# mit-han-lab/duo-attention

Hardware: NVIDIA H100
Metric: decode tok/s @512K ctx (+ prefill tok/s @128K in `prefill`), Llama-3-8B, DuoAttention 50% retrieval heads (higher is better)
Workload: dtype bf16

## Files before the change

duo_attention_b200/_C.py:

```python
from __future__ import annotations

import ctypes as C
import os

_HERE = os.path.dirname(os.path.abspath(__file__))
LIB_PATH = os.environ.get("DUO_B200_LIB") or os.path.join(_HERE, "csrc", "libduo_b200.so")

DUO_OK, DUO_EINVAL, DUO_EOVERFLOW, DUO_ECUDA, DUO_EWORKSPACE = 0, -1, -2, -3, -4
DT_BF16, DT_FP16 = 0, 1
KV_SAME, KV_INT4 = 0, 1
ROPE_NONE, ROPE_HF, ROPE_FP32 = 0, 1, 2
ROPE_SKIP_Q = 0x100
DECODE_MAX_Q = 16
DECODE_MAX_Q_INT4 = 8
RAGGED_MAX_BATCH = 64

SYMBOLS = [
    "duo_layer_create", "duo_layer_destroy", "duo_workspace_bytes", "duo_rope_append", "duo_attention",
    "duo_attention_mma", "duo_decode_fused", "duo_decode_ragged", "duo_ragged_workspace_bytes",
    "duo_decode_ragged_int4", "duo_ragged_int4_workspace_bytes", "duo_layer_create_pooled", "duo_decode_ragged_pooled",
    "duo_ragged_state_advance", "duo_state_advance", "duo_state_set", "duo_stream_commit", "duo_quant_int4", "duo_dequant_int4", "duo_dequant_int4_bf16", "duo_add_rmsnorm", "duo_silu_mul",
    "duo_attention_partial", "duo_merge_partials", "duo_attention_seq", "duo_decode_fused_seq",
    "duo_seqcomm_data_bytes", "duo_seqcomm_flag_bytes", "duo_seqcomm_create", "duo_seqcomm_destroy", "duo_seq_merge",
    "duo_comm_data_bytes", "duo_comm_flag_bytes", "duo_comm_create", "duo_comm_destroy", "duo_allreduce_add_rmsnorm",
    "duo_last_error_string", "duo_version",
]


class LayerDesc(C.Structure):
    _fields_ = [
        ("full_k", C.c_void_p), ("full_v", C.c_void_p), ("ring_k", C.c_void_p), ("ring_v", C.c_void_p),
        ("full_k_scale", C.c_void_p), ("full_k_zero", C.c_void_p), ("full_v_scale", C.c_void_p),
        ("full_v_zero", C.c_void_p), ("ring_k_scale", C.c_void_p), ("ring_k_zero", C.c_void_p),
        ("ring_v_scale", C.c_void_p), ("ring_v_zero", C.c_void_p),
        ("full_cap", C.c_int64),
        ("batch", C.c_int32), ("n_full", C.c_int32), ("n_stream", C.c_int32), ("group", C.c_int32),
        ("head_dim", C.c_int32), ("sink", C.c_int32), ("recent", C.c_int32), ("stage_cap", C.c_int32),
        ("dtype", C.c_int32), ("kv_format", C.c_int32),
    ]


class CacheState(C.Structure):
    _fields_ = [("full_len", C.c_int64), ("total", C.c_int64), ("lo", C.c_int64), ("device_state", C.c_void_p),
                ("seq_rank", C.c_int32), ("seq_world", C.c_int32), ("seq_block", C.c_int32), ("seq_reserved", C.c_int32)]


class SeqCommDesc(C.Structure):
    _fields_ = [("data", C.c_void_p * 8), ("flags", C.c_void_p * 8), ("local_state", C.c_void_p),
                ("rank", C.c_int32), ("world", C.c_int32), ("max_rows", C.c_int32)]


class CommDesc(C.Structure):
    _fields_ = [("data", C.c_void_p * 8), ("flags", C.c_void_p * 8), ("local_state", C.c_void_p),
                ("rank", C.c_int32), ("world", C.c_int32), ("hidden", C.c_int32), ("max_rows", C.c_int32),
                ("dtype", C.c_int32)]


_lib = None


def load():
    global _lib
    if _lib is not None:
        return _lib
    if not os.path.exists(LIB_PATH):
        raise RuntimeError(
            f"{LIB_PATH} not found: the CUDA extension is mandatory (no fallback). Build it with "
            "`python -c 'import __graft_entry__ as g; g.build()'` or `make -C duo_attention_b200/csrc`."
        )
    lib = C.CDLL(LIB_PATH)
    vp, i32, i64, f32, sz = C.c_void_p, C.c_int32, C.c_int64, C.c_float, C.c_size_t
    lib.duo_layer_create.argtypes = [C.POINTER(LayerDesc), C.POINTER(vp)]
    lib.duo_layer_create.restype = C.c_int
    lib.duo_layer_create_pooled.argtypes = [C.POINTER(LayerDesc), i64, C.POINTER(vp)]
    lib.duo_layer_create_pooled.restype = C.c_int
    lib.duo_layer_destroy.argtypes = [vp]
    lib.duo_layer_destroy.restype = None
    lib.duo_workspace_bytes.argtypes = [i32, i32, i32, i32]
    lib.duo_workspace_bytes.restype = sz
    lib.duo_rope_append.argtypes = [vp, C.POINTER(CacheState), vp, i64, vp, vp, i32, i32, vp]
    lib.duo_rope_append.restype = C.c_int
    for name in ("duo_attention", "duo_attention_mma"):
        fn = getattr(lib, name)
        fn.argtypes = [vp, C.POINTER(CacheState), vp, i64, vp, i32, f32, vp, sz, vp]
        fn.restype = C.c_int
    lib.duo_decode_fused.argtypes = [vp, C.POINTER(CacheState), vp, i64, vp, vp, i32, vp, i32, f32, vp, sz, vp]
    lib.duo_decode_fused.restype = C.c_int
    for name in ("duo_decode_ragged", "duo_decode_ragged_int4"):
        fn = getattr(lib, name)
        fn.argtypes = [vp, vp, i64, vp, i64, vp, vp, i32, vp, i32, f32, vp, sz, vp]
        fn.restype = C.c_int
    lib.duo_decode_ragged_pooled.argtypes = [vp, vp, vp, i64, vp, i64, vp, vp, i32, vp, i32, f32, vp, sz, vp]
    lib.duo_decode_ragged_pooled.restype = C.c_int
    for name in ("duo_ragged_workspace_bytes", "duo_ragged_int4_workspace_bytes"):
        fn = getattr(lib, name)
        fn.argtypes = [i32, i32]
        fn.restype = sz
    lib.duo_ragged_state_advance.argtypes = [vp, i32, i32, i32, i32, vp]
    lib.duo_ragged_state_advance.restype = C.c_int
    lib.duo_state_advance.argtypes = [vp, i32, i32, i32, vp]
    lib.duo_state_advance.restype = C.c_int
    lib.duo_state_set.argtypes = [vp, i64, i64, i64, vp]
    lib.duo_state_set.restype = C.c_int
    lib.duo_stream_commit.argtypes = [vp, C.POINTER(CacheState), i32, vp]
    lib.duo_stream_commit.restype = C.c_int
    lib.duo_quant_int4.argtypes = [vp, i64, i64, vp, vp, vp, vp]
    lib.duo_quant_int4.restype = C.c_int
    for name in ("duo_dequant_int4", "duo_dequant_int4_bf16"):
        fn = getattr(lib, name)
        fn.argtypes = [vp, vp, vp, i64, vp, vp]
        fn.restype = C.c_int
    lib.duo_add_rmsnorm.argtypes = [vp, vp, vp, vp, vp, i64, i32, f32, i32, vp]
    lib.duo_add_rmsnorm.restype = C.c_int
    lib.duo_silu_mul.argtypes = [vp, vp, i64, i32, i32, vp]
    lib.duo_silu_mul.restype = C.c_int
    lib.duo_attention_partial.argtypes = [vp, i64, vp, i64, vp, vp, i32, f32, vp, sz, vp]
    lib.duo_attention_partial.restype = C.c_int
    lib.duo_attention_seq.argtypes = [vp, C.POINTER(CacheState), vp, i64, vp, vp, vp, i32, f32, vp, sz, vp]
    lib.duo_attention_seq.restype = C.c_int
    lib.duo_decode_fused_seq.argtypes = [vp, C.POINTER(CacheState), vp, i64, vp, vp, i32, vp, vp, vp, f32, vp, sz, vp]
    lib.duo_decode_fused_seq.restype = C.c_int
    lib.duo_seqcomm_data_bytes.argtypes = [i32, i32]
    lib.duo_seqcomm_data_bytes.restype = sz
    lib.duo_seqcomm_flag_bytes.argtypes = [i32, i32]
    lib.duo_seqcomm_flag_bytes.restype = sz
    lib.duo_seqcomm_create.argtypes = [C.POINTER(SeqCommDesc), C.POINTER(vp)]
    lib.duo_seqcomm_create.restype = C.c_int
    lib.duo_seqcomm_destroy.argtypes = [vp]
    lib.duo_seqcomm_destroy.restype = None
    lib.duo_seq_merge.argtypes = [vp, vp, vp, vp, i32, i32, i32, i32, vp]
    lib.duo_seq_merge.restype = C.c_int
    lib.duo_merge_partials.argtypes = [vp, vp, i32, i64, i32, i32, vp, i32, vp]
    lib.duo_merge_partials.restype = C.c_int
    lib.duo_comm_data_bytes.argtypes = [i32, i32, i32, i32]
    lib.duo_comm_data_bytes.restype = sz
    lib.duo_comm_flag_bytes.argtypes = [i32, i32]
    lib.duo_comm_flag_bytes.restype = sz
    lib.duo_comm_create.argtypes = [C.POINTER(CommDesc), C.POINTER(vp)]
    lib.duo_comm_create.restype = C.c_int
    lib.duo_comm_destroy.argtypes = [vp]
    lib.duo_comm_destroy.restype = None
    lib.duo_allreduce_add_rmsnorm.argtypes = [vp, vp, vp, vp, vp, vp, i32, f32, vp]
    lib.duo_allreduce_add_rmsnorm.restype = C.c_int
    lib.duo_last_error_string.argtypes = []
    lib.duo_last_error_string.restype = C.c_char_p
    lib.duo_version.argtypes = []
    lib.duo_version.restype = C.c_int
    _lib = lib
    return lib


def last_error() -> str:
    return load().duo_last_error_string().decode("utf-8", "replace")


def check(rc: int):
    if rc == DUO_OK:
        return
    msg = last_error()
    if rc == DUO_EOVERFLOW or rc == DUO_EINVAL:
        raise ValueError(msg)
    raise RuntimeError(f"libduo_b200 error {rc}: {msg}")
```

duo_attention_b200/csrc/api.cu:

```cuda
#include <cstdarg>
#include <cstdio>
#include <cstdlib>
#include <cstring>
#include <new>

#include "duo_common.cuh"

namespace duo {

int sm_count_current_device() {
  static int sms[64] = {0};
  int dev = 0;
  if (cudaGetDevice(&dev) != cudaSuccess) return 132;
  int& v = sms[dev & 63];
  if (v == 0) {
    int n = 132;
    if (cudaDeviceGetAttribute(&n, cudaDevAttrMultiProcessorCount, dev) != cudaSuccess || n < 1) n = 132;
    v = n;
  }
  return v;
}

static thread_local char g_err[512] = "";

void set_error(const char* fmt, ...) {
  va_list ap;
  va_start(ap, fmt);
  vsnprintf(g_err, sizeof(g_err), fmt, ap);
  va_end(ap);
}
int cuda_fail(cudaError_t e, const char* what) {
  set_error("CUDA error %d (%s) in %s", (int)e, cudaGetErrorString(e), what);
  return DUO_ECUDA;
}

size_t mma_workspace_bytes(int batch, int n_kv, int group, int max_q_len);
int launch_attn_mma(const duo_layer* L, const duo_cache_state* st, const void* q, long long q_row_stride, void* out,
                    int q_len, float scale, void* workspace, size_t workspace_bytes, cudaStream_t stream);
int launch_attn_int4(const duo_layer* L, const duo_cache_state* st, const void* q, long long q_row_stride, void* out,
                     int q_len, float scale, void* workspace, size_t workspace_bytes, cudaStream_t stream);
bool tc_prefill_supported(const duo_layer* L, const duo_cache_state* st, int q_len);
int launch_attn_tc(const duo_layer* L, const duo_cache_state* st, const void* q, long long q_row_stride, void* out,
                   int q_len, float scale, cudaStream_t stream);
int launch_rope_append(const duo_layer* L, const duo_cache_state* st, void* qkv, long long row_stride, const void* cos,
                       const void* sin, int rope_mode, int q_len, cudaStream_t stream);
int launch_stream_commit(const duo_layer* L, const duo_cache_state* st, int q_len, cudaStream_t stream);
int launch_quant_int4(const void* in, long long in_row_stride, long long rows, void* packed, void* scale, void* zero,
                      cudaStream_t stream);
int launch_state_advance(long long* st, int n, int sink, int recent, cudaStream_t stream);
int launch_state_set(long long* st, long long full_len, long long total, long long lo, cudaStream_t stream);
int launch_dequant_int4(const void* packed, const void* scale, const void* zero, long long rows, void* out,
                        cudaStream_t stream);
int launch_dequant_int4_bf16(const void* packed, const void* scale, const void* zero, long long rows, void* out,
                             cudaStream_t stream);

int launch_attn_mma_partial(const duo_layer* L, long long n_keys, const void* q, long long q_row_stride, float* out_o,
                            float* out_lse, int q_len, float scale, void* workspace, size_t workspace_bytes,
                            cudaStream_t stream);
int launch_attn_mma_seq(const duo_layer* L, const duo_cache_state* st, const void* q, long long q_row_stride, void* out,
                        float* part_o, float* part_lse, int q_len, float scale, void* workspace, size_t workspace_bytes,
                        cudaStream_t stream);
int launch_decode_fused(const duo_layer* L, const duo_cache_state* st, const void* qkv, long long row_stride,
                        const void* cos, const void* sin, int rope_mode, void* out, int q_len, float scale,
                        void* workspace, size_t workspace_bytes, cudaStream_t stream);
int launch_decode_fused_int4(const duo_layer* L, const duo_cache_state* st, const void* qkv, long long row_stride,
                             const void* cos, const void* sin, int rope_mode, void* out, int q_len, float scale,
                             void* workspace, size_t workspace_bytes, cudaStream_t stream);
int launch_decode_ragged(const duo_layer* L, const long long* row_state, const long long* row_geom, const void* qkv,
                         long long row_stride, const void* cos, const void* sin, int rope_mode, void* out, int q_len,
                         float scale, void* workspace, size_t workspace_bytes, cudaStream_t stream);
size_t ragged_workspace_bytes(int batch, int n_kv);
int launch_decode_ragged_int4(const duo_layer* L, const long long* row_state, const long long* row_geom,
                              const void* qkv, long long row_stride, const void* cos, const void* sin, int rope_mode,
                              void* out, int q_len, float scale, void* workspace, size_t workspace_bytes,
                              cudaStream_t stream);
size_t ragged_int4_workspace_bytes(int batch, int n_kv);
int launch_ragged_state_advance(long long* st, int batch, int n, int sink, int recent, cudaStream_t stream);
int launch_decode_fused_seq(const duo_layer* L, const duo_cache_state* st, const void* qkv, long long row_stride,
                            const void* cos, const void* sin, int rope_mode, void* out, float* part_o, float* part_lse,
                            float scale, void* workspace, size_t workspace_bytes, cudaStream_t stream);
int launch_merge_partials(const float* o_parts, const float* lse_parts, int n_parts, long long tokens, int heads_total,
                          int heads_used, void* out, int dtype, cudaStream_t stream);
int launch_add_rmsnorm(const void* x, const void* residual, const void* weight, void* out_norm, void* out_res,
                       long long rows, int hidden, float eps, int dtype, cudaStream_t stream);
int launch_silu_mul(const void* gate_up, void* out, long long rows, int inter, int dtype, cudaStream_t stream);

typedef CUresult (*EncodeTiledFn)(CUtensorMap*, CUtensorMapDataType, cuuint32_t, void*, const cuuint64_t*,
                                  const cuuint64_t*, const cuuint32_t*, const cuuint32_t*, CUtensorMapInterleave,
                                  CUtensorMapSwizzle, CUtensorMapL2promotion, CUtensorMapFloatOOBfill);

EncodeTiledFn get_encode_fn() {
  static EncodeTiledFn fn = nullptr;
  if (fn) return fn;
  void* p = nullptr;
  cudaDriverEntryPointQueryResult qres;
  cudaError_t e = cudaGetDriverEntryPoint("cuTensorMapEncodeTiled", &p, cudaEnableDefault, &qres);
  if (e != cudaSuccess || qres != cudaDriverEntryPointSuccess || p == nullptr) {
    set_error("cudaGetDriverEntryPoint(cuTensorMapEncodeTiled) failed: %s", cudaGetErrorString(e));
    cudaGetLastError();
    return nullptr;
  }
  fn = reinterpret_cast<EncodeTiledFn>(p);
  return fn;
}

static int encode_kv_map(CUtensorMap* m, void* base, int dtype, long long slots, long long heads, int box_rows) {
  EncodeTiledFn fn = get_encode_fn();
  if (!fn) return DUO_ECUDA;
  cuuint64_t dims[3] = {(cuuint64_t)kHeadDim, (cuuint64_t)slots, (cuuint64_t)heads};
  cuuint64_t strides[2] = {(cuuint64_t)kHeadDim * 2, (cuuint64_t)slots * kHeadDim * 2};
  cuuint32_t box[3] = {64, (cuuint32_t)box_rows, 1};
  cuuint32_t estr[3] = {1, 1, 1};
  CUresult r = fn(m, dtype == DUO_DT_BF16 ? CU_TENSOR_MAP_DATA_TYPE_BFLOAT16 : CU_TENSOR_MAP_DATA_TYPE_FLOAT16, 3, base,
                  dims, strides, box, estr, CU_TENSOR_MAP_INTERLEAVE_NONE, CU_TENSOR_MAP_SWIZZLE_128B,
                  CU_TENSOR_MAP_L2_PROMOTION_L2_256B, CU_TENSOR_MAP_FLOAT_OOB_FILL_NONE);
  if (r != CUDA_SUCCESS) {
    set_error("cuTensorMapEncodeTiled failed with CUresult %d (base=%p slots=%lld heads=%lld)", (int)r, base, slots,
              heads);
    return DUO_ECUDA;
  }
  return DUO_OK;
}

int stage_offset(const duo_layer_desc& d) {
  const int W = d.sink + d.recent;
  return d.kv_format == DUO_KV_INT4 ? (W + 63) / 64 * 64 : W;
}

}

using namespace duo;

extern "C" {

const char* duo_last_error_string(void) { return g_err; }
int duo_version(void) { return 100; }

static int create_layer(const duo_layer_desc* desc, int64_t pool_tokens, duo_layer** out) {
  *out = nullptr;
  if (desc->head_dim != kHeadDim) {
    set_error("duo_layer_create: head_dim %d unsupported (only 128)", desc->head_dim);
    return DUO_EINVAL;
  }
  if (desc->batch < 1 || desc->n_full < 0 || desc->n_stream < 0 || desc->group < 1 || desc->sink < 0 ||
      desc->recent < 1 || desc->stage_cap < 1 || desc->full_cap < 0) {
    set_error("duo_layer_create: bad geometry");
    return DUO_EINVAL;
  }
  if (desc->dtype != DUO_DT_BF16 && desc->dtype != DUO_DT_FP16) {
    set_error("duo_layer_create: bad dtype %d", desc->dtype);
    return DUO_EINVAL;
  }
  if (desc->kv_format == DUO_KV_INT4) {
    const long long ring_slots = (long long)stage_offset(*desc) + desc->stage_cap;
    if ((pool_tokens == 0 && desc->full_cap % 8 != 0) || ring_slots % 8 != 0) {
      set_error("duo_layer_create: INT4 caches need full_cap and ring slots (%lld) to be multiples of 8", ring_slots);
      return DUO_EINVAL;
    }
  }
  duo_layer* L = new (std::nothrow) duo_layer();
  if (!L) {
    set_error("duo_layer_create: out of host memory");
    return DUO_EINVAL;
  }
  L->d = *desc;
  L->has_full_maps = false;
  L->has_ring_maps = false;
  L->pool_tokens = pool_tokens;
  memset(&L->maps, 0, sizeof(L->maps));
  if (desc->kv_format == DUO_KV_SAME) {
    const long long ring_slots = (long long)desc->sink + desc->recent + desc->stage_cap;
    int rc = DUO_OK;
    const long long slots = pool_tokens ? pool_tokens * desc->n_full : desc->full_cap;
    if (desc->n_full > 0 && slots > 0) {
      const long long heads = pool_tokens ? 1 : (long long)desc->batch * desc->n_full;
      rc = encode_kv_map(&L->maps.full_k64, desc->full_k, desc->dtype, slots, heads, 64);
      if (!rc) rc = encode_kv_map(&L->maps.full_v64, desc->full_v, desc->dtype, slots, heads, 64);
      if (!rc) rc = encode_kv_map(&L->maps.full_k128, desc->full_k, desc->dtype, slots, heads, 128);
      if (!rc) rc = encode_kv_map(&L->maps.full_v128, desc->full_v, desc->dtype, slots, heads, 128);
      L->has_full_maps = (rc == DUO_OK);
    }
    if (!rc && desc->n_stream > 0) {
      const long long heads = (long long)desc->batch * desc->n_stream;
      rc = encode_kv_map(&L->maps.ring_k64, desc->ring_k, desc->dtype, ring_slots, heads, 64);
      if (!rc) rc = encode_kv_map(&L->maps.ring_v64, desc->ring_v, desc->dtype, ring_slots, heads, 64);
      if (!rc) rc = encode_kv_map(&L->maps.ring_k128, desc->ring_k, desc->dtype, ring_slots, heads, 128);
      if (!rc) rc = encode_kv_map(&L->maps.ring_v128, desc->ring_v, desc->dtype, ring_slots, heads, 128);
      L->has_ring_maps = (rc == DUO_OK);
    }
    if (rc) {
      delete L;
      return rc;
    }
  }
  *out = L;
  return DUO_OK;
}

int duo_layer_create(const duo_layer_desc* desc, duo_layer** out) {
  if (!desc || !out) {
    set_error("duo_layer_create: null argument");
    return DUO_EINVAL;
  }
  return create_layer(desc, 0, out);
}

int duo_layer_create_pooled(const duo_layer_desc* desc, int64_t pool_tokens, duo_layer** out) {
  if (!desc || !out) {
    set_error("duo_layer_create_pooled: null argument");
    return DUO_EINVAL;
  }
  *out = nullptr;
  if (pool_tokens < 128 || pool_tokens % 128 != 0) {
    set_error("duo_layer_create_pooled: pool_tokens %lld is not a positive multiple of 128", (long long)pool_tokens);
    return DUO_EINVAL;
  }
  if (desc->n_full > 0 && pool_tokens * desc->n_full > INT32_MAX) {
    set_error("duo_layer_create_pooled: pool of %lld tokens x %d retrieval heads exceeds the 32-bit TMA row coordinate",
              (long long)pool_tokens, desc->n_full);
    return DUO_EINVAL;
  }
  return create_layer(desc, pool_tokens, out);
}

void duo_layer_destroy(duo_layer* layer) { delete layer; }

size_t duo_workspace_bytes(int32_t batch, int32_t n_kv_heads, int32_t group, int32_t max_q_len) {
  return mma_workspace_bytes(batch, n_kv_heads, group, max_q_len);
}

static int check_chunk(const duo_layer* L, const duo_cache_state* st, int q_len, const char* who) {
  if (!L || !st) {
    set_error("%s: null layer/state", who);
    return DUO_EINVAL;
  }
  if (L->pool_tokens) {
    set_error("%s: a pooled ragged layer is decoded with duo_decode_ragged_pooled only", who);
    return DUO_EINVAL;
  }
  if (q_len < 1) {
    set_error("%s: q_len %d < 1", who, q_len);
    return DUO_EINVAL;
  }
  if (st->full_len < 0 || st->total < 0 || st->lo < 0) {
    set_error("%s: negative cache state", who);
    return DUO_EINVAL;
  }
  long long need = st->full_len + q_len;
  if (st->seq_world != 0) {
    if (st->seq_world < 2 || st->seq_world > 8 || st->seq_rank < 0 || st->seq_rank >= st->seq_world || st->seq_block < 1) {
      set_error("%s: bad sequence-shard descriptor (rank %d, world %d, block %d)", who, st->seq_rank, st->seq_world,
                st->seq_block);
      return DUO_EINVAL;
    }
    const long long round = (long long)st->seq_block * st->seq_world, rem = need % round;
    long long extra = rem - (long long)st->seq_rank * st->seq_block;
    extra = extra < 0 ? 0 : (extra > st->seq_block ? st->seq_block : extra);
    need = need / round * st->seq_block + extra;
  }
  if (L->d.n_full > 0 && need > L->d.full_cap) {
    set_error("Trying to put %d KVs into a cache with max size %lld, current size: %lld.", q_len,
              (long long)L->d.full_cap, (long long)st->full_len);
    return DUO_EOVERFLOW;
  }
  if (q_len > L->d.stage_cap) {
    set_error("%s: chunk of %d tokens exceeds the staging capacity %d", who, q_len, L->d.stage_cap);
    return DUO_EOVERFLOW;
  }
  return DUO_OK;
}

int duo_rope_append(const duo_layer* layer, const duo_cache_state* st, void* qkv, int64_t qkv_row_stride,
                    const void* cos, const void* sin, int32_t rope_mode, int32_t q_len, void* stream) {
  int rc = check_chunk(layer, st, q_len, "duo_rope_append");
  if (rc) return rc;
  if (!qkv || ((rope_mode & 0xff) != DUO_ROPE_NONE && (!cos || !sin))) {
    set_error("duo_rope_append: null buffer");
    return DUO_EINVAL;
  }
  if ((rope_mode & 0xff) < DUO_ROPE_NONE || (rope_mode & 0xff) > DUO_ROPE_FP32 || (rope_mode & ~(0xff | DUO_ROPE_SKIP_Q))) {
    set_error("duo_rope_append: bad rope_mode %d", rope_mode);
    return DUO_EINVAL;
  }
  if (qkv_row_stride % 4 != 0) {
    set_error("duo_rope_append: row stride must be a multiple of 4 elements");
    return DUO_EINVAL;
  }
  return launch_rope_append(layer, st, qkv, qkv_row_stride, cos, sin, rope_mode, q_len, (cudaStream_t)stream);
}

int duo_attention(const duo_layer* layer, const duo_cache_state* st, const void* q, int64_t q_row_stride, void* out,
                  int32_t q_len, float scale, void* workspace, size_t workspace_bytes, void* stream) {
  int rc = check_chunk(layer, st, q_len, "duo_attention");
  if (rc) return rc;
  if (!q || !out) {
    set_error("duo_attention: null buffer");
    return DUO_EINVAL;
  }
  if (st->seq_world != 0) {
    set_error("duo_attention: sequence-sharded caches are attended with duo_attention_seq");
    return DUO_EINVAL;
  }
  if (layer->d.kv_format == DUO_KV_INT4)
    return launch_attn_int4(layer, st, q, q_row_stride, out, q_len, scale, workspace, workspace_bytes,
                            (cudaStream_t)stream);
  if (st->device_state && q_len > DUO_DECODE_MAX_Q) {
    set_error("duo_attention: device_state is only supported for chunks of <= %d tokens", DUO_DECODE_MAX_Q);
    return DUO_EINVAL;
  }
  if (tc_prefill_supported(layer, st, q_len))
    return launch_attn_tc(layer, st, q, q_row_stride, out, q_len, scale, (cudaStream_t)stream);
  return launch_attn_mma(layer, st, q, q_row_stride, out, q_len, scale, workspace, workspace_bytes,
                         (cudaStream_t)stream);
}

static int check_decode_args(const char* who, bool outputs_ok, const void* qkv, int64_t qkv_row_stride, const void* cos,
                             const void* sin, int32_t rope_mode) {
  if (!outputs_ok || !qkv || (rope_mode != DUO_ROPE_NONE && (!cos || !sin))) {
    set_error("%s: null buffer", who);
    return DUO_EINVAL;
  }
  if (rope_mode < DUO_ROPE_NONE || rope_mode > DUO_ROPE_FP32) {
    set_error("%s: bad rope_mode %d", who, rope_mode);
    return DUO_EINVAL;
  }
  if (qkv_row_stride % 8 != 0 || (reinterpret_cast<uintptr_t>(qkv) & 15)) {
    set_error("%s: qkv rows must be 16-byte aligned (row stride a multiple of 8 elements)", who);
    return DUO_EINVAL;
  }
  return DUO_OK;
}

int duo_decode_fused(const duo_layer* layer, const duo_cache_state* st, const void* qkv, int64_t qkv_row_stride,
                     const void* cos, const void* sin, int32_t rope_mode, void* out, int32_t q_len, float scale,
                     void* workspace, size_t workspace_bytes, void* stream) {
  int rc = check_chunk(layer, st, q_len, "duo_decode_fused");
  if (!rc) rc = check_decode_args("duo_decode_fused", out != nullptr, qkv, qkv_row_stride, cos, sin, rope_mode);
  if (rc) return rc;
  const int max_rows = layer->d.kv_format == DUO_KV_INT4 ? DUO_DECODE_MAX_Q_INT4 : DUO_DECODE_MAX_Q;
  if (layer->d.group * q_len > max_rows || st->seq_world != 0) {
    set_error("duo_decode_fused: unsharded caches and group * q_len <= %d only (got group %d, q_len %d)", max_rows,
              layer->d.group, q_len);
    return DUO_EINVAL;
  }
  if (layer->d.kv_format == DUO_KV_INT4)
    return launch_decode_fused_int4(layer, st, qkv, qkv_row_stride, cos, sin, rope_mode, out, q_len, scale, workspace,
                                    workspace_bytes, (cudaStream_t)stream);
  return launch_decode_fused(layer, st, qkv, qkv_row_stride, cos, sin, rope_mode, out, q_len, scale, workspace,
                             workspace_bytes, (cudaStream_t)stream);
}

size_t duo_ragged_workspace_bytes(int32_t batch, int32_t n_kv_heads) {
  if (batch < 1 || batch > DUO_RAGGED_MAX_BATCH || n_kv_heads < 1) return 0;
  return ragged_workspace_bytes(batch, n_kv_heads);
}

size_t duo_ragged_int4_workspace_bytes(int32_t batch, int32_t n_kv_heads) {
  if (batch < 1 || batch > DUO_RAGGED_MAX_BATCH || n_kv_heads < 1) return 0;
  return ragged_int4_workspace_bytes(batch, n_kv_heads);
}

static int check_ragged_rows(const char* who, const duo_layer* layer, int32_t q_len, int max_rows) {
  if (layer->d.batch > DUO_RAGGED_MAX_BATCH) {
    set_error("%s: batch %d exceeds %d rows", who, layer->d.batch, DUO_RAGGED_MAX_BATCH);
    return DUO_EINVAL;
  }
  if (q_len < 1 || layer->d.group * q_len > max_rows) {
    set_error("%s: group * q_len <= %d only (got group %d, q_len %d)", who, max_rows, layer->d.group, q_len);
    return DUO_EINVAL;
  }
  return DUO_OK;
}

static int check_ragged_args(const char* who, const duo_layer* layer, int64_t max_full_len, int32_t q_len,
                             int max_rows) {
  if (int rc = check_ragged_rows(who, layer, q_len, max_rows)) return rc;
  if (max_full_len < 0) {
    set_error("%s: negative max_full_len", who);
    return DUO_EINVAL;
  }
  if (layer->d.n_full > 0 && max_full_len + q_len > layer->d.full_cap) {
    set_error("Trying to put %d KVs into a cache with max size %lld, current size: %lld.", q_len,
              (long long)layer->d.full_cap, (long long)max_full_len);
    return DUO_EOVERFLOW;
  }
  return DUO_OK;
}

int duo_decode_ragged(const duo_layer* layer, const int64_t* row_state, int64_t max_full_len, const void* qkv,
                      int64_t qkv_row_stride, const void* cos, const void* sin, int32_t rope_mode, void* out,
                      int32_t q_len, float scale, void* workspace, size_t workspace_bytes, void* stream) {
  if (!layer || !row_state) {
    set_error("duo_decode_ragged: null argument");
    return DUO_EINVAL;
  }
  if (layer->pool_tokens) {
    set_error("duo_decode_ragged: a pooled ragged layer is decoded with duo_decode_ragged_pooled");
    return DUO_EINVAL;
  }
  if (int rc = check_decode_args("duo_decode_ragged", out != nullptr, qkv, qkv_row_stride, cos, sin, rope_mode)) return rc;
  if (layer->d.kv_format != DUO_KV_SAME) {
    set_error("duo_decode_ragged: 16-bit KV only (INT4 caches are decoded with duo_decode_ragged_int4)");
    return DUO_EINVAL;
  }
  if (int rc = check_ragged_args("duo_decode_ragged", layer, max_full_len, q_len, DUO_DECODE_MAX_Q)) return rc;
  return launch_decode_ragged(layer, reinterpret_cast<const long long*>(row_state), nullptr, qkv, qkv_row_stride, cos,
                              sin, rope_mode, out, q_len, scale, workspace, workspace_bytes, (cudaStream_t)stream);
}

int duo_decode_ragged_int4(const duo_layer* layer, const int64_t* row_state, int64_t max_full_len, const void* qkv,
                           int64_t qkv_row_stride, const void* cos, const void* sin, int32_t rope_mode, void* out,
                           int32_t q_len, float scale, void* workspace, size_t workspace_bytes, void* stream) {
  if (!layer || !row_state) {
    set_error("duo_decode_ragged_int4: null argument");
    return DUO_EINVAL;
  }
  if (layer->pool_tokens) {
    set_error("duo_decode_ragged_int4: a pooled ragged layer is decoded with duo_decode_ragged_pooled");
    return DUO_EINVAL;
  }
  if (int rc = check_decode_args("duo_decode_ragged_int4", out != nullptr, qkv, qkv_row_stride, cos, sin, rope_mode))
    return rc;
  if (layer->d.kv_format != DUO_KV_INT4) {
    set_error("duo_decode_ragged_int4: INT4 caches only (16-bit caches are decoded with duo_decode_ragged)");
    return DUO_EINVAL;
  }
  if (int rc = check_ragged_args("duo_decode_ragged_int4", layer, max_full_len, q_len, DUO_DECODE_MAX_Q_INT4)) return rc;
  return launch_decode_ragged_int4(layer, reinterpret_cast<const long long*>(row_state), nullptr, qkv, qkv_row_stride,
                                   cos, sin, rope_mode, out, q_len, scale, workspace, workspace_bytes,
                                   (cudaStream_t)stream);
}

int duo_decode_ragged_pooled(const duo_layer* layer, const int64_t* row_state, const int64_t* row_geom,
                             int64_t min_room, const void* qkv, int64_t qkv_row_stride, const void* cos,
                             const void* sin, int32_t rope_mode, void* out, int32_t q_len, float scale,
                             void* workspace, size_t workspace_bytes, void* stream) {
  const char* who = "duo_decode_ragged_pooled";
  if (!layer || !row_state || !row_geom) {
    set_error("%s: null argument", who);
    return DUO_EINVAL;
  }
  if (int rc = check_decode_args(who, out != nullptr, qkv, qkv_row_stride, cos, sin, rope_mode)) return rc;
  if (!layer->pool_tokens) {
    set_error("%s: the layer has no retrieval pool (create it with duo_layer_create_pooled)", who);
    return DUO_EINVAL;
  }
  const bool int4 = layer->d.kv_format == DUO_KV_INT4;
  if (int rc = check_ragged_rows(who, layer, q_len, int4 ? DUO_DECODE_MAX_Q_INT4 : DUO_DECODE_MAX_Q)) return rc;
  if (layer->d.n_full > 0 && q_len > min_room) {
    set_error("Trying to put %d KVs into a cache row with room for %lld more (%s).", q_len, (long long)min_room, who);
    return DUO_EOVERFLOW;
  }
  const long long* rs = reinterpret_cast<const long long*>(row_state);
  const long long* rg = reinterpret_cast<const long long*>(row_geom);
  if (int4)
    return launch_decode_ragged_int4(layer, rs, rg, qkv, qkv_row_stride, cos, sin, rope_mode, out, q_len, scale,
                                     workspace, workspace_bytes, (cudaStream_t)stream);
  return launch_decode_ragged(layer, rs, rg, qkv, qkv_row_stride, cos, sin, rope_mode, out, q_len, scale, workspace,
                              workspace_bytes, (cudaStream_t)stream);
}

int duo_ragged_state_advance(int64_t* row_state, int32_t batch, int32_t n, int32_t sink, int32_t recent, void* stream) {
  if (!row_state || batch < 1 || batch > DUO_RAGGED_MAX_BATCH || n < 0 || recent < 1 || sink < 0) {
    set_error("duo_ragged_state_advance: bad argument");
    return DUO_EINVAL;
  }
  return launch_ragged_state_advance(reinterpret_cast<long long*>(row_state), batch, n, sink, recent,
                                     (cudaStream_t)stream);
}

int duo_decode_fused_seq(const duo_layer* layer, const duo_cache_state* st, const void* qkv, int64_t qkv_row_stride,
                         const void* cos, const void* sin, int32_t rope_mode, void* out, float* out_o, float* out_lse,
                         float scale, void* workspace, size_t workspace_bytes, void* stream) {
  int rc = check_chunk(layer, st, 1, "duo_decode_fused_seq");
  if (!rc)
    rc = check_decode_args("duo_decode_fused_seq", out && out_o && out_lse, qkv, qkv_row_stride, cos, sin, rope_mode);
  if (rc) return rc;
  if (st->seq_world < 2) {
    set_error("duo_decode_fused_seq: the cache state carries no sequence-shard descriptor");
    return DUO_EINVAL;
  }
  if (layer->d.kv_format != DUO_KV_SAME || layer->d.group > 16) {
    set_error("duo_decode_fused_seq: 16-bit caches and group <= 16 only");
    return DUO_EINVAL;
  }
  return launch_decode_fused_seq(layer, st, qkv, qkv_row_stride, cos, sin, rope_mode, out, out_o, out_lse, scale, workspace,
                                 workspace_bytes, (cudaStream_t)stream);
}

int duo_attention_mma(const duo_layer* layer, const duo_cache_state* st, const void* q, int64_t q_row_stride,
                      void* out, int32_t q_len, float scale, void* workspace, size_t workspace_bytes, void* stream) {
  int rc = check_chunk(layer, st, q_len, "duo_attention_mma");
  if (rc) return rc;
  if (layer->d.kv_format != DUO_KV_SAME) {
    set_error("duo_attention_mma: 16-bit KV only");
    return DUO_EINVAL;
  }
  return launch_attn_mma(layer, st, q, q_row_stride, out, q_len, scale, workspace, workspace_bytes,
                         (cudaStream_t)stream);
}

int duo_state_advance(int64_t* device_state, int32_t n, int32_t sink, int32_t recent, void* stream) {
  if (!device_state || n < 0 || recent < 1 || sink < 0) {
    set_error("duo_state_advance: bad argument");
    return DUO_EINVAL;
  }
  return launch_state_advance(reinterpret_cast<long long*>(device_state), n, sink, recent, (cudaStream_t)stream);
}

int duo_state_set(int64_t* device_state, int64_t full_len, int64_t total, int64_t lo, void* stream) {
  if (!device_state || full_len < 0 || total < 0 || lo < 0) {
    set_error("duo_state_set: bad argument");
    return DUO_EINVAL;
  }
  return launch_state_set(reinterpret_cast<long long*>(device_state), full_len, total, lo, (cudaStream_t)stream);
}

int duo_stream_commit(const duo_layer* layer, const duo_cache_state* st, int32_t q_len, void* stream) {
  int rc = check_chunk(layer, st, q_len, "duo_stream_commit");
  if (rc) return rc;
  return launch_stream_commit(layer, st, q_len, (cudaStream_t)stream);
}

int duo_quant_int4(const void* in, int64_t in_row_stride, int64_t rows, void* packed, void* scale, void* zero,
                   void* stream) {
  if (rows < 0 || (rows > 0 && (!in || !packed || !scale || !zero)) || in_row_stride % 4 != 0) {
    set_error("duo_quant_int4: bad argument");
    return DUO_EINVAL;
  }
  return launch_quant_int4(in, in_row_stride, rows, packed, scale, zero, (cudaStream_t)stream);
}

int duo_attention_partial(const duo_layer* layer, int64_t n_keys, const void* q, int64_t q_row_stride, float* out_o,
                          float* out_lse, int32_t q_len, float scale, void* workspace, size_t workspace_bytes,
                          void* stream) {
  if (!layer || !q || !out_o || !out_lse || n_keys < 0 || q_len < 1) {
    set_error("duo_attention_partial: bad argument");
    return DUO_EINVAL;
  }
  if (layer->pool_tokens) {
    set_error("duo_attention_partial: a pooled ragged layer is decoded with duo_decode_ragged_pooled only");
    return DUO_EINVAL;
  }
  if (layer->d.kv_format != DUO_KV_SAME || layer->d.group * q_len > 16) {
    set_error("duo_attention_partial: 16-bit caches and group * q_len <= 16 only (got group %d, q_len %d)",
              layer->d.group, q_len);
    return DUO_EINVAL;
  }
  if (layer->d.n_full > 0 && n_keys > layer->d.full_cap) {
    set_error("duo_attention_partial: n_keys %lld exceeds the cache capacity %lld", (long long)n_keys,
              (long long)layer->d.full_cap);
    return DUO_EOVERFLOW;
  }
  return launch_attn_mma_partial(layer, n_keys, q, q_row_stride, out_o, out_lse, q_len, scale, workspace,
                                 workspace_bytes, (cudaStream_t)stream);
}

int duo_attention_seq(const duo_layer* layer, const duo_cache_state* st, const void* q, int64_t q_row_stride, void* out,
                      float* out_o, float* out_lse, int32_t q_len, float scale, void* workspace, size_t workspace_bytes,
                      void* stream) {
  int rc = check_chunk(layer, st, q_len, "duo_attention_seq");
  if (rc) return rc;
  if (!q || !out || !out_o || !out_lse) {
    set_error("duo_attention_seq: null buffer");
    return DUO_EINVAL;
  }
  if (st->seq_world < 2) {
    set_error("duo_attention_seq: the cache state carries no sequence-shard descriptor");
    return DUO_EINVAL;
  }
  if (layer->d.kv_format != DUO_KV_SAME || layer->d.group * q_len > 16) {
    set_error("duo_attention_seq: 16-bit caches and group * q_len <= 16 only (got group %d, q_len %d)", layer->d.group,
              q_len);
    return DUO_EINVAL;
  }
  return launch_attn_mma_seq(layer, st, q, q_row_stride, out, out_o, out_lse, q_len, scale, workspace, workspace_bytes,
                             (cudaStream_t)stream);
}

int duo_merge_partials(const float* o_parts, const float* lse_parts, int32_t n_parts, int64_t tokens,
                       int32_t heads_total, int32_t heads_used, void* out, int32_t dtype, void* stream) {
  if (n_parts < 1 || tokens < 0 || heads_total < 1 || heads_used < 0 || heads_used > heads_total ||
      (tokens > 0 && heads_used > 0 && (!o_parts || !lse_parts || !out)) ||
      (dtype != DUO_DT_BF16 && dtype != DUO_DT_FP16)) {
    set_error("duo_merge_partials: bad argument");
    return DUO_EINVAL;
  }
  return launch_merge_partials(o_parts, lse_parts, n_parts, tokens, heads_total, heads_used, out, dtype,
                               (cudaStream_t)stream);
}

int duo_add_rmsnorm(const void* x, const void* residual, const void* weight, void* out_norm, void* out_res, int64_t rows,
                    int32_t hidden, float eps, int32_t dtype, void* stream) {
  if (rows < 0 || hidden < 8 || hidden % 8 != 0 || hidden > 16384 || (rows > 0 && (!x || !weight || !out_norm)) ||
      (dtype != DUO_DT_BF16 && dtype != DUO_DT_FP16)) {
    set_error("duo_add_rmsnorm: bad argument");
    return DUO_EINVAL;
  }
  return launch_add_rmsnorm(x, residual, weight, out_norm, out_res, rows, hidden, eps, dtype, (cudaStream_t)stream);
}

int duo_silu_mul(const void* gate_up, void* out, int64_t rows, int32_t inter, int32_t dtype, void* stream) {
  if (rows < 0 || inter < 8 || inter % 8 != 0 || (rows > 0 && (!gate_up || !out)) ||
      (dtype != DUO_DT_BF16 && dtype != DUO_DT_FP16)) {
    set_error("duo_silu_mul: bad argument");
    return DUO_EINVAL;
  }
  return launch_silu_mul(gate_up, out, rows, inter, dtype, (cudaStream_t)stream);
}

int duo_dequant_int4(const void* packed, const void* scale, const void* zero, int64_t rows, void* out, void* stream) {
  if (rows < 0 || (rows > 0 && (!packed || !scale || !zero || !out))) {
    set_error("duo_dequant_int4: bad argument");
    return DUO_EINVAL;
  }
  return launch_dequant_int4(packed, scale, zero, rows, out, (cudaStream_t)stream);
}

int duo_dequant_int4_bf16(const void* packed, const void* scale, const void* zero, int64_t rows, void* out,
                          void* stream) {
  if (rows < 0 || (rows > 0 && (!packed || !scale || !zero || !out))) {
    set_error("duo_dequant_int4_bf16: bad argument");
    return DUO_EINVAL;
  }
  return launch_dequant_int4_bf16(packed, scale, zero, rows, out, (cudaStream_t)stream);
}

}
```

duo_attention_b200/csrc/attn_mma.cu:

```cuda
#include <type_traits>

#include "duo_common.cuh"

namespace duo {

constexpr int TILE = 64;
constexpr int STAGES = 3;
constexpr int KV_BOX_BYTES = TILE * 128;
constexpr int STAGE_BYTES = 4 * KV_BOX_BYTES;
constexpr int ATTN_THREADS = 128;

struct AttnParams {
  const void* q;
  void* out;
  long long q_tok_stride;
  long long q_batch_stride;
  long long out_batch_stride;
  int q_len, n_q_heads, group, n_full, n_stream, batch;
  int sink, recent, W;
  long long full_len, total, lo;
  const long long* dstate;
  float scale_log2;
  int splits_full;
  int keys_per_split;
  int n_rb;
  int cache_scan;
  SplitWs ws;
  float* part_o;
  float* part_lse;
  int no_causal;
  int seq_rank, seq_world, seq_block;
  const void* cos;
  const void* sin;
  int rope_mode;
  long long k_off, v_off;
  void *full_k, *full_v, *ring_k, *ring_v;
  long long full_cap;
  int ring_slots;
  int rg_slots;
  int rg_want;
  const long long* row_geom;
};


__host__ __device__ __forceinline__ long long seq_local_len(long long n, int rank, int world, int block) {
  const long long round = (long long)block * world;
  const long long full_rounds = n / round, rem = n % round;
  long long extra = rem - (long long)rank * block;
  extra = extra < 0 ? 0 : (extra > block ? block : extra);
  return full_rounds * block + extra;
}

template <typename T>
__device__ __forceinline__ void rope2(uint32_t& lo2, uint32_t& hi2, const void* cos, const void* sin, int mode, int tok,
                                      int d) {
  T* xl = reinterpret_cast<T*>(&lo2);
  T* xh = reinterpret_cast<T*>(&hi2);
#pragma unroll
  for (int e = 0; e < 2; ++e) {
    const float a = RopeCvt<T>::to_f(xl[e]), bb = RopeCvt<T>::to_f(xh[e]);
    float ol, oh;
    if (mode == DUO_ROPE_HF) {
      const T* ct = reinterpret_cast<const T*>(cos) + (long long)tok * kHeadDim;
      const T* st = reinterpret_cast<const T*>(sin) + (long long)tok * kHeadDim;
      ol = rope_hf<T>(a, -bb, RopeCvt<T>::to_f(ct[d + e]), RopeCvt<T>::to_f(st[d + e]));
      oh = rope_hf<T>(bb, a, RopeCvt<T>::to_f(ct[d + 64 + e]), RopeCvt<T>::to_f(st[d + 64 + e]));
    } else {
      const float* ct = reinterpret_cast<const float*>(cos) + (long long)tok * kHeadDim;
      const float* st = reinterpret_cast<const float*>(sin) + (long long)tok * kHeadDim;
      ol = rope_f32(a, -bb, ct[d + e], st[d + e]);
      oh = rope_f32(bb, a, ct[d + 64 + e], st[d + 64 + e]);
    }
    xl[e] = RopeCvt<T>::from_f(ol);
    xh[e] = RopeCvt<T>::from_f(oh);
  }
}

#ifdef DUO_TRACE
__device__ unsigned long long* g_duo_trace_mma = nullptr;
__device__ __forceinline__ void trace_stamp_mma(int slot) {
  if (threadIdx.x == 0 && g_duo_trace_mma) {
    unsigned long long t;
    asm volatile("mov.u64 %0, %%globaltimer;" : "=l"(t));
    g_duo_trace_mma[((long long)blockIdx.y * gridDim.x + blockIdx.x) * 4 + slot] = t;
  }
}
#define DUO_TRACE_MMA(slot) trace_stamp_mma(slot)
#else
#define DUO_TRACE_MMA(slot)
#endif

template <typename T, int KEY_WARPS, bool FUSED, bool RAGGED = false, bool POOLED = false>
__global__ void __launch_bounds__(ATTN_THREADS, 2)
duo_attn_mma_kernel(const __grid_constant__ CUtensorMap map_fk, const __grid_constant__ CUtensorMap map_fv,
                    const __grid_constant__ CUtensorMap map_rk, const __grid_constant__ CUtensorMap map_rv,
                    const AttnParams pin) {
  static_assert(!RAGGED || (FUSED && KEY_WARPS == 4), "the ragged variant is the fused decode kernel");
  static_assert(!POOLED || RAGGED, "the pooled layout is a ragged decode layout");
  DUO_TRACE_MMA(0);
  AttnParams p = pin;
  if (!RAGGED && pin.dstate) {
    p.full_len = pin.dstate[0];
    p.total = pin.dstate[1];
    p.lo = pin.dstate[2];
    const long long nk = p.seq_world > 1
                             ? seq_local_len(p.full_len + (FUSED ? 0 : p.q_len), p.seq_rank, p.seq_world, p.seq_block)
                             : p.full_len + (FUSED ? 0 : p.q_len);
    p.keys_per_split = (int)split_keys(nk, p.splits_full, TILE);
    p.cache_scan = (int)(p.total < p.W ? p.total : p.W);
  }
  constexpr int ROW_WARPS = 4 / KEY_WARPS;
  constexpr int ROWS = 16 * ROW_WARPS;
  constexpr int KPW = TILE / KEY_WARPS;
  constexpr int NT = KPW / 8;
  using Op = MmaOp<T>;

  extern __shared__ __align__(1024) uint8_t smem_raw[];
  uint8_t* smem = reinterpret_cast<uint8_t*>((reinterpret_cast<uintptr_t>(smem_raw) + 1023) & ~uintptr_t(1023));
  __shared__ uint64_t full_bar[STAGES];
  __shared__ int s_is_last;
  __shared__ float s_wmax[2][4][16];

  const int tid = threadIdx.x;
  const int warp = tid >> 5, lane = tid & 31;
  const int g = lane >> 2, t4 = lane & 3;
  int b = blockIdx.y;

  const int n_full_items = p.n_full * p.n_rb * p.splits_full;
  int kvh, rb, split;
  bool is_full;
  if constexpr (RAGGED) {
    const long long* rs = pin.dstate;
    rb = 0;
    split = 0;
    const int x = blockIdx.x, n_fslots = p.n_full * p.rg_slots;
    is_full = x < n_fslots;
    if (is_full) {
      const long long kps = ragged_batch_kps(rs, p.batch, 0, p.rg_want, TILE, 4 * TILE);
      kvh = x / p.rg_slots;
      const RaggedSlot s = ragged_slot(rs, p.batch, 0, kps, x % p.rg_slots);
      b = s.b;
      if (b == p.batch) return;
      split = s.split;
      p.keys_per_split = (int)kps;
      p.splits_full = s.splits;
      ragged_ws_slice<16>(p.ws, b, kvh, p.n_full, p.rg_slots, s);
    } else {
      const int y = x - n_fslots;
      b = y / p.n_stream;
      kvh = p.n_full + y % p.n_stream;
    }
    p.full_len = rs[4 * b];
    p.total = rs[4 * b + 1];
    p.lo = rs[4 * b + 2];
    p.cache_scan = (int)(p.total < p.W ? p.total : p.W);
    const long long tab = (long long)b * p.q_len * kHeadDim * (p.rope_mode == DUO_ROPE_HF ? (long long)sizeof(T) : 4);
    p.cos = reinterpret_cast<const uint8_t*>(p.cos) + tab;
    p.sin = reinterpret_cast<const uint8_t*>(p.sin) + tab;
  } else if ((int)blockIdx.x < n_full_items) {
    is_full = true;
    int x = blockIdx.x;
    split = x % p.splits_full;
    x /= p.splits_full;
    rb = p.n_rb - 1 - (x % p.n_rb);
    kvh = x / p.n_rb;
  } else {
    is_full = false;
    int x = blockIdx.x - n_full_items;
    rb = p.n_rb - 1 - (x % p.n_rb);
    kvh = p.n_full + x / p.n_rb;
    split = 0;
  }
  const int rows_total = p.group * p.q_len;
  const int row0 = rb * ROWS;
  const int rows_here = min(ROWS, rows_total - row0);
  const int tok_max = (row0 + rows_here - 1) / p.group;

  long long a0, a1, b0 = 0, b1 = 0;
  auto vis_count = [&](int t) -> long long {
    if (!is_full) return (long long)p.W + t + 1;
    if (p.no_causal) return p.full_len;
    if (p.seq_world > 1) return seq_local_len(p.full_len + t + 1, p.seq_rank, p.seq_world, p.seq_block);
    return p.full_len + t + 1;
  };
  bool has_new = false;
  long long new_base = 0;
  if (is_full) {
    const long long cached = p.seq_world > 1 ? seq_local_len(p.full_len, p.seq_rank, p.seq_world, p.seq_block) : p.full_len;
    const long long nkeys = FUSED ? cached : vis_count(tok_max);
    a0 = (long long)split * p.keys_per_split;
    a1 = min(nkeys, a0 + (long long)p.keys_per_split);
    if (a1 < a0) a1 = a0;
    has_new = FUSED && (split == p.splits_full - 1);
    if (FUSED && p.seq_world > 1)
      has_new = has_new && ((int)((p.full_len / p.seq_block) % p.seq_world) == p.seq_rank);
    new_base = cached;
  } else {
    a0 = 0;
    a1 = p.cache_scan;
    b0 = p.W;
    b1 = FUSED ? b0 : (long long)p.W + tok_max + 1;
    has_new = FUSED;
    new_base = p.W;
  }
  const int nA = (int)((a1 - a0 + TILE - 1) / TILE);
  const int nB = (int)((b1 - b0 + TILE - 1) / TILE);
  const int n_tiles = nA + nB;
  const int n_iter = n_tiles + (has_new ? 1 : 0);
  const CUtensorMap* mk = is_full ? &map_fk : &map_rk;
  const CUtensorMap* mv = is_full ? &map_fv : &map_rv;
  int pool_row0 = 0;
  if constexpr (POOLED) {
    if (is_full) pool_row0 = (int)(pin.row_geom[2 * b] * p.n_full + kvh * pin.row_geom[2 * b + 1]);
  }
  const int head_coord = (POOLED && is_full) ? 0 : is_full ? (b * p.n_full + kvh) : (b * p.n_stream + (kvh - p.n_full));

  if (tid == 0) {
    prefetch_tmap(mk);
    prefetch_tmap(mv);
    for (int s = 0; s < STAGES; ++s) mbar_init(&full_bar[s], 1);
    fence_barrier_init();
  }
  __syncthreads();

  auto tile_start = [&](int i) -> long long { return i < nA ? a0 + (long long)i * TILE : b0 + (long long)(i - nA) * TILE; };
  auto issue = [&](int i) {
    const int s = i % STAGES;
    uint8_t* dst = smem + s * STAGE_BYTES;
    const int j0 = (int)tile_start(i) + (POOLED ? pool_row0 : 0);
    mbar_expect_tx(&full_bar[s], STAGE_BYTES);
    tma_load_3d(dst, mk, &full_bar[s], 0, j0, head_coord);
    tma_load_3d(dst + KV_BOX_BYTES, mk, &full_bar[s], 64, j0, head_coord);
    tma_load_3d(dst + 2 * KV_BOX_BYTES, mv, &full_bar[s], 0, j0, head_coord);
    tma_load_3d(dst + 3 * KV_BOX_BYTES, mv, &full_bar[s], 64, j0, head_coord);
  };
  if (tid == 0) {
    for (int i = 0; i < STAGES - 1 && i < n_tiles; ++i) issue(i);
  }

  const int wrow = (KEY_WARPS == 1) ? warp * 16 : 0;
  const int wkey = (KEY_WARPS == 1) ? 0 : warp * KPW;
  uint32_t qa[8][4];
  int tok_r[2];
  {
    const T* qb = reinterpret_cast<const T*>(p.q) + (long long)b * p.q_batch_stride;
#pragma unroll
    for (int hf = 0; hf < 2; ++hf) {
      const int R = row0 + wrow + g + hf * 8;
      const bool ok = R < rows_total;
      const int tok = ok ? R / p.group : 0;
      const int hq = kvh * p.group + (ok ? R % p.group : 0);
      tok_r[hf] = ok ? tok : -1;
      const T* src = qb + (long long)tok * p.q_tok_stride + (long long)hq * kHeadDim;
#pragma unroll
      for (int kk = 0; kk < 8; ++kk) {
        uint32_t v0 = 0, v1 = 0;
        if (ok) {
          v0 = *reinterpret_cast<const uint32_t*>(src + kk * 16 + 2 * t4);
          v1 = *reinterpret_cast<const uint32_t*>(src + kk * 16 + 8 + 2 * t4);
        }
        qa[kk][hf] = v0;
        qa[kk][hf + 2] = v1;
      }
      if constexpr (FUSED) {
        if (ok && p.rope_mode != DUO_ROPE_NONE) {
#pragma unroll
          for (int kk = 0; kk < 4; ++kk) {
#pragma unroll
            for (int half = 0; half < 2; ++half) {
              const int d = kk * 16 + half * 8 + 2 * t4;
              rope2<T>(qa[kk][hf + 2 * half], qa[kk + 4][hf + 2 * half], p.cos, p.sin, p.rope_mode, tok, d);
            }
          }
        }
      }
    }
  }

  const long long lim_r[2] = {tok_r[0] >= 0 ? vis_count(tok_r[0]) : 0, tok_r[1] >= 0 ? vis_count(tok_r[1]) : 0};
  const long long lim_min = vis_count((row0 + wrow) / p.group);

  float o[16][4];
#pragma unroll
  for (int i = 0; i < 16; ++i) o[i][0] = o[i][1] = o[i][2] = o[i][3] = 0.f;
  float m_run[2] = {-INFINITY, -INFINITY};
  float l_run[2] = {0.f, 0.f};

  const int lrow = lane & 7;
  const int lmat = lane >> 3;

  for (int i = 0; i < n_iter; ++i) {
    __syncthreads();
    uint32_t sK;
    long long j0, jend;
    if (!FUSED || i < n_tiles) {
      if (tid == 0 && i + STAGES - 1 < n_tiles) issue(i + STAGES - 1);
      const int s = i % STAGES;
      mbar_wait(&full_bar[s], (i / STAGES) & 1);
      sK = smem_u32(smem + s * STAGE_BYTES);
      j0 = tile_start(i);
      jend = (i < nA) ? a1 : b1;
    } else {
      uint8_t* st0 = smem;
      for (int x = tid; x < STAGE_BYTES / 16; x += ATTN_THREADS) reinterpret_cast<uint4*>(st0)[x] = make_uint4(0, 0, 0, 0);
      __syncthreads();
      const T* rows = reinterpret_cast<const T*>(p.q) + (long long)b * p.q_batch_stride;
      auto dst_row = [&](int r) -> long long {
        if (is_full)
          return (POOLED ? (long long)pool_row0 : ((long long)b * p.n_full + kvh) * p.full_cap) + new_base + r;
        const long long pos = p.total + r;
        long long slot;
        if (pos < p.sink) slot = pos;
        else if (r >= p.q_len - p.recent) slot = p.sink + (pos - p.sink) % p.recent;
        else return -1;
        return ((long long)b * p.n_stream + (kvh - p.n_full)) * p.ring_slots + slot;
      };
      T* gk = reinterpret_cast<T*>(is_full ? p.full_k : p.ring_k);
      T* gv = reinterpret_cast<T*>(is_full ? p.full_v : p.ring_v);
      for (int w = tid; w < p.q_len * 8; w += ATTN_THREADS) {
        const int r = w >> 3, c = w & 7;
        const T* src = rows + (long long)r * p.q_tok_stride + p.k_off + (long long)kvh * kHeadDim;
        uint4 lo = *reinterpret_cast<const uint4*>(src + c * 8);
        uint4 hi = *reinterpret_cast<const uint4*>(src + 64 + c * 8);
        if (p.rope_mode != DUO_ROPE_NONE) rope8<T>(lo, hi, p.cos, p.sin, p.rope_mode, r, c * 8);
        const uint32_t off = r * 128 + ((c ^ (r & 7)) << 4);
        *reinterpret_cast<uint4*>(st0 + off) = lo;
        *reinterpret_cast<uint4*>(st0 + KV_BOX_BYTES + off) = hi;
        const long long dr = dst_row(r);
        if (dr >= 0) {
          *reinterpret_cast<uint4*>(gk + dr * kHeadDim + c * 8) = lo;
          *reinterpret_cast<uint4*>(gk + dr * kHeadDim + 64 + c * 8) = hi;
        }
      }
      for (int w = tid; w < p.q_len * 16; w += ATTN_THREADS) {
        const int r = w >> 4, c = w & 15;
        const T* src = rows + (long long)r * p.q_tok_stride + p.v_off + (long long)kvh * kHeadDim;
        const uint4 v = *reinterpret_cast<const uint4*>(src + c * 8);
        *reinterpret_cast<uint4*>(st0 + (2 + (c >> 3)) * KV_BOX_BYTES + r * 128 + (((c & 7) ^ (r & 7)) << 4)) = v;
        const long long dr = dst_row(r);
        if (dr >= 0) *reinterpret_cast<uint4*>(gv + dr * kHeadDim + c * 8) = v;
      }
      __syncthreads();
      sK = smem_u32(st0);
      j0 = new_base;
      jend = new_base + p.q_len;
    }
    const uint32_t sV = sK + 2 * KV_BOX_BYTES;

    float sc[NT][4];
#pragma unroll
    for (int n = 0; n < NT; ++n) sc[n][0] = sc[n][1] = sc[n][2] = sc[n][3] = 0.f;
#pragma unroll
    for (int kk = 0; kk < 8; ++kk) {
#pragma unroll
      for (int pr = 0; pr < NT / 2; ++pr) {
        const int krow = wkey + pr * 16 + (lmat >> 1) * 8 + lrow;
        const int cc = kk * 2 + (lmat & 1);
        const uint32_t addr = sK + (cc >> 3) * KV_BOX_BYTES + krow * 128 + (((cc & 7) ^ (krow & 7)) << 4);
        uint32_t r0, r1, r2, r3;
        ldsm_x4(r0, r1, r2, r3, addr);
        Op::run(sc[2 * pr], qa[kk], r0, r1);
        Op::run(sc[2 * pr + 1], qa[kk], r2, r3);
      }
    }

    const long long kfirst = j0 + wkey;
    const bool need_mask = (kfirst + KPW > jend) || (kfirst + KPW > lim_min) ||
                           (!is_full && i < nA);
    if (need_mask) {
#pragma unroll
      for (int n = 0; n < NT; ++n) {
#pragma unroll
        for (int e = 0; e < 4; ++e) {
          const long long j = kfirst + n * 8 + 2 * t4 + (e & 1);
          bool vis = (j < jend) && (j < lim_r[e >> 1]);
          if (!is_full && j < p.W) vis = vis && stream_slot_valid((int)j, p.sink, p.recent, p.total, p.lo);
          if (!vis) sc[n][e] = -INFINITY;
        }
      }
    }
    float mx[2] = {-INFINITY, -INFINITY};
#pragma unroll
    for (int n = 0; n < NT; ++n) {
      mx[0] = fmaxf(mx[0], fmaxf(sc[n][0], sc[n][1]));
      mx[1] = fmaxf(mx[1], fmaxf(sc[n][2], sc[n][3]));
    }
#pragma unroll
    for (int hf = 0; hf < 2; ++hf) {
      mx[hf] = fmaxf(mx[hf], __shfl_xor_sync(0xffffffffu, mx[hf], 1));
      mx[hf] = fmaxf(mx[hf], __shfl_xor_sync(0xffffffffu, mx[hf], 2));
    }
    if constexpr (KEY_WARPS == 4) {
      if (n_iter <= 8) {
        if (t4 == 0) {
          s_wmax[i & 1][warp][g] = mx[0];
          s_wmax[i & 1][warp][g + 8] = mx[1];
        }
        __syncthreads();
#pragma unroll
        for (int w = 0; w < 4; ++w) {
          mx[0] = fmaxf(mx[0], s_wmax[i & 1][w][g]);
          mx[1] = fmaxf(mx[1], s_wmax[i & 1][w][g + 8]);
        }
      }
    }
    float alpha[2], msc[2];
#pragma unroll
    for (int hf = 0; hf < 2; ++hf) {
      const float m_new = fmaxf(m_run[hf], mx[hf]);
      msc[hf] = (m_new == -INFINITY) ? 0.f : m_new * p.scale_log2;
      alpha[hf] = (m_run[hf] == -INFINITY) ? 0.f : fast_exp2(m_run[hf] * p.scale_log2 - msc[hf]);
      m_run[hf] = m_new;
    }
    float rs[2] = {0.f, 0.f};
    uint32_t pa[NT / 2][4];
#pragma unroll
    for (int n = 0; n < NT; ++n) {
      const float p0 = fast_exp2(sc[n][0] * p.scale_log2 - msc[0]);
      const float p1 = fast_exp2(sc[n][1] * p.scale_log2 - msc[0]);
      const float p2 = fast_exp2(sc[n][2] * p.scale_log2 - msc[1]);
      const float p3 = fast_exp2(sc[n][3] * p.scale_log2 - msc[1]);
      rs[0] += p0 + p1;
      rs[1] += p2 + p3;
      pa[n >> 1][(n & 1) * 2 + 0] = Op::pack(p0, p1);
      pa[n >> 1][(n & 1) * 2 + 1] = Op::pack(p2, p3);
    }
#pragma unroll
    for (int hf = 0; hf < 2; ++hf) l_run[hf] = l_run[hf] * alpha[hf] + rs[hf];
#pragma unroll
    for (int d = 0; d < 16; ++d) {
      o[d][0] *= alpha[0];
      o[d][1] *= alpha[0];
      o[d][2] *= alpha[1];
      o[d][3] *= alpha[1];
    }

#pragma unroll
    for (int k2 = 0; k2 < NT / 2; ++k2) {
#pragma unroll
      for (int q2 = 0; q2 < 8; ++q2) {
        const int krow = wkey + k2 * 16 + (lmat & 1) * 8 + lrow;
        const int cc = q2 * 2 + (lmat >> 1);
        const uint32_t addr = sV + (cc >> 3) * KV_BOX_BYTES + krow * 128 + (((cc & 7) ^ (krow & 7)) << 4);
        uint32_t r0, r1, r2, r3;
        ldsm_x4_trans(r0, r1, r2, r3, addr);
        Op::run(o[2 * q2], pa[k2], r0, r1);
        Op::run(o[2 * q2 + 1], pa[k2], r2, r3);
      }
    }
  }

  DUO_TRACE_MMA(1);
#pragma unroll
  for (int hf = 0; hf < 2; ++hf) {
    l_run[hf] += __shfl_xor_sync(0xffffffffu, l_run[hf], 1);
    l_run[hf] += __shfl_xor_sync(0xffffffffu, l_run[hf], 2);
  }

  __syncthreads();
  float* sm_o = reinterpret_cast<float*>(smem);
  float* sm_ml = reinterpret_cast<float*>(smem + 64 * 1024);
  if constexpr (KEY_WARPS == 4) {
    float* w_o = reinterpret_cast<float*>(smem) + 16 * 128;
    float* w_ml = sm_ml + 64;
#pragma unroll
    for (int hf = 0; hf < 2; ++hf) {
      const int r = g + hf * 8;
      if (t4 == 0) {
        w_ml[(warp * 16 + r) * 2 + 0] = (m_run[hf] == -INFINITY) ? -INFINITY : m_run[hf] * p.scale_log2;
        w_ml[(warp * 16 + r) * 2 + 1] = l_run[hf];
      }
#pragma unroll
      for (int d = 0; d < 16; ++d) {
        float2 v = make_float2(o[d][hf * 2], o[d][hf * 2 + 1]);
        *reinterpret_cast<float2*>(&w_o[(warp * 16 + r) * 128 + d * 8 + 2 * t4]) = v;
      }
    }
    __syncthreads();
    for (int idx = tid; idx < 16 * 128; idx += ATTN_THREADS) {
      const int r = idx >> 7, d = idx & 127;
      float mm = -INFINITY;
#pragma unroll
      for (int w = 0; w < 4; ++w) mm = fmaxf(mm, w_ml[(w * 16 + r) * 2]);
      float acc = 0.f, ll = 0.f;
#pragma unroll
      for (int w = 0; w < 4; ++w) {
        const float mw = w_ml[(w * 16 + r) * 2];
        const float f = (mw == -INFINITY) ? 0.f : fast_exp2(mw - mm);
        acc += f * w_o[(w * 16 + r) * 128 + d];
        ll += f * w_ml[(w * 16 + r) * 2 + 1];
      }
      sm_o[r * 128 + d] = acc;
      if (d == 0) {
        sm_ml[r * 2] = mm;
        sm_ml[r * 2 + 1] = ll;
      }
    }
  } else {
#pragma unroll
    for (int hf = 0; hf < 2; ++hf) {
      const int r = wrow + g + hf * 8;
      if (t4 == 0) {
        sm_ml[r * 2 + 0] = (m_run[hf] == -INFINITY) ? -INFINITY : m_run[hf] * p.scale_log2;
        sm_ml[r * 2 + 1] = l_run[hf];
      }
#pragma unroll
      for (int d = 0; d < 16; ++d) {
        float2 v = make_float2(o[d][hf * 2], o[d][hf * 2 + 1]);
        *reinterpret_cast<float2*>(&sm_o[r * 128 + d * 8 + 2 * t4]) = v;
      }
    }
  }
  __syncthreads();

  T* outb = reinterpret_cast<T*>(p.out) + (long long)b * p.out_batch_stride;
  auto store_row_elem = [&](int r, int d, float v0, float v1) {
    const int R = row0 + r;
    const int tok = R / p.group;
    const int hq = kvh * p.group + R % p.group;
    if (p.part_o && is_full) {
      float* dst = p.part_o + (((long long)b * p.q_len + tok) * p.n_q_heads + hq) * kHeadDim + d;
      *reinterpret_cast<float2*>(dst) = make_float2(v0, v1);
      return;
    }
    T* dst = outb + ((long long)tok * p.n_q_heads + hq) * kHeadDim + d;
    *reinterpret_cast<uint32_t*>(dst) = Op::pack(v0, v1);
  };
  auto store_row_lse = [&](int r, float m_log2, float l) {
    const int R = row0 + r;
    p.part_lse[((long long)b * p.q_len + R / p.group) * p.n_q_heads + kvh * p.group + R % p.group] =
        l > 0.f ? m_log2 + log2f(l) : -INFINITY;
  };

  const int nsplit = is_full ? p.splits_full : 1;
  if (nsplit == 1) {
    for (int idx = tid; idx < rows_here * 64; idx += ATTN_THREADS) {
      const int r = idx >> 6, d = (idx & 63) * 2;
      const float l = sm_ml[r * 2 + 1];
      const float inv = l > 0.f ? 1.f / l : 0.f;
      store_row_elem(r, d, sm_o[r * 128 + d] * inv, sm_o[r * 128 + d + 1] * inv);
      if (p.part_lse && is_full && d == 0) store_row_lse(r, sm_ml[r * 2], l);
    }
    return;
  }

  const long long item = RAGGED ? 0 : ((long long)b * p.n_full + kvh) * p.n_rb + rb;
  float* wo = p.ws.ws_o + (item * p.splits_full + split) * (long long)(ROWS * 128);
  float* wml = p.ws.ws_ml + (item * p.splits_full + split) * (long long)(ROWS * 2);
  for (int idx = tid; idx < rows_here * 32; idx += ATTN_THREADS) {
    const int r = idx >> 5, d4 = (idx & 31) * 4;
    *reinterpret_cast<float4*>(&wo[r * 128 + d4]) = *reinterpret_cast<const float4*>(&sm_o[r * 128 + d4]);
  }
  if (tid < rows_here * 2) wml[tid] = sm_ml[tid];
  DUO_TRACE_MMA(2);
  split_kv_finish<ROWS>(p.ws, item, split, p.splits_full, rows_here, reinterpret_cast<float*>(smem),
                        reinterpret_cast<float*>(smem + 80 * 1024), &s_is_last,
                        [&](int r, int d, float v0, float v1, float mm, float ll) {
                          store_row_elem(r, d, v0, v1);
                          if (p.part_lse && d == 0) store_row_lse(r, mm, ll);
                        });
  DUO_TRACE_MMA(3);
}

constexpr int ATTN_SMEM_BYTES = STAGES * STAGE_BYTES + 1024;

size_t mma_workspace_bytes(int batch, int n_kv, int group, int max_q_len) {
  const long long max_partials = 4 * 160 + 64;
  const long long rows = (long long)group * max_q_len;
  const long long items = (long long)batch * n_kv * ((rows + 15) / 16);
  const long long l1 = max_partials * 64 * 130 * 4;
  const long long l2 = (max_partials / kMergeGroup + items + 8) * 64 * 130 * 4;
  return (size_t)(kSplitCounterBytes + l1 + l2 + 8192);
}

struct PartialMode {
  float* part_o = nullptr;
  float* part_lse = nullptr;
  bool no_causal = false;
};
int stage_offset(const duo_layer_desc& d);

static void fill_fused(AttnParams& p, const duo_layer_desc& d, const FusedArgs& fa) {
  fill_fused_args(p, fa);
  p.full_k = d.full_k;
  p.full_v = d.full_v;
  p.ring_k = d.ring_k;
  p.ring_v = d.ring_v;
  p.full_cap = d.full_cap;
  p.ring_slots = stage_offset(d) + d.stage_cap;
}

template <typename T, int KEY_WARPS, bool FUSED, bool RAGGED = false, bool POOLED = false>
static int launch_mma_kernel(const duo_layer* L, dim3 grid, const AttnParams& p, cudaStream_t stream) {
  if (grid.x == 0) return DUO_OK;
  auto kern = duo_attn_mma_kernel<T, KEY_WARPS, FUSED, RAGGED, POOLED>;
  static unsigned long long attr_mask = 0;
  if (int rc = ensure_dyn_smem(kern, ATTN_SMEM_BYTES, &attr_mask)) return rc;
  const KvMaps m = kv_maps(L, false);
  kern<<<grid, ATTN_THREADS, ATTN_SMEM_BYTES, stream>>>(*m.fk, *m.fv, *m.rk, *m.rv, p);
  DUO_CUDA_TRY(cudaGetLastError());
  return DUO_OK;
}

template <typename T, int KEY_WARPS, bool FUSED = false>
static int launch_variant(const duo_layer* L, const duo_cache_state* st, const void* q, long long q_row_stride,
                          void* out, int q_len, float scale, void* workspace, size_t workspace_bytes,
                          cudaStream_t stream, PartialMode pm = PartialMode(), FusedArgs fa = FusedArgs()) {
  const duo_layer_desc& d = L->d;
  constexpr int ROWS = 16 * (4 / KEY_WARPS);
  AttnParams p{};
  fill_common_params(p, d, *st, q, q_row_stride, out, q_len, scale);
  if (FUSED) fill_fused(p, d, fa);
  p.n_rb = (d.group * q_len + ROWS - 1) / ROWS;
  const bool partial = pm.no_causal;
  p.part_o = pm.part_o;
  p.part_lse = pm.part_lse;
  p.no_causal = pm.no_causal ? 1 : 0;
  p.seq_rank = st->seq_rank;
  p.seq_world = st->seq_world;
  p.seq_block = st->seq_block;

  const long long seen = (partial || FUSED) ? st->full_len : st->full_len + q_len;
  const long long nkeys = (!partial && st->seq_world > 1) ? seq_local_len(seen, st->seq_rank, st->seq_world, st->seq_block)
                                                          : seen;
  const int full_ctas = d.batch * d.n_full * p.n_rb, stream_ctas = partial ? 0 : d.batch * d.n_stream * p.n_rb;
  const SplitPlan sp = plan_splits(nkeys, 2 * sm_count_current_device(), full_ctas, stream_ctas, TILE, 4 * TILE);
  p.splits_full = sp.splits;
  p.keys_per_split = (int)sp.keys_per_split;
  if (sp.splits > 1)
    if (int rc = split_ws_carve(p.ws, split_ws_layout(full_ctas, sp.splits, ROWS), workspace, workspace_bytes,
                                "duo_attention"))
      return rc;

  const int grid_x = d.n_full * p.n_rb * sp.splits + (partial ? 0 : d.n_stream * p.n_rb);
  return launch_mma_kernel<T, KEY_WARPS, FUSED>(L, dim3(grid_x, d.batch), p, stream);
}

int launch_attn_mma(const duo_layer* L, const duo_cache_state* st, const void* q, long long q_row_stride, void* out,
                    int q_len, float scale, void* workspace, size_t workspace_bytes, cudaStream_t stream) {
  const bool decode_rows = L->d.group * q_len <= 16;
  return dispatch_dtype(L->d.dtype, [&](auto t) {
    using T = decltype(t);
    return decode_rows ? launch_variant<T, 4>(L, st, q, q_row_stride, out, q_len, scale, workspace, workspace_bytes, stream)
                       : launch_variant<T, 1>(L, st, q, q_row_stride, out, q_len, scale, workspace, workspace_bytes, stream);
  });
}

template <typename T>
__global__ void __launch_bounds__(128) merge_partials_kernel(const float* __restrict__ o_parts,
                                                             const float* __restrict__ lse_parts, int n_parts,
                                                             long long tokens, int heads_total, int heads_used,
                                                             T* __restrict__ out) {
  const long long tok = blockIdx.x / heads_used;
  const int h = (int)(blockIdx.x % heads_used);
  const long long row = tok * heads_total + h;
  const long long part_rows = tokens * heads_total;
  float mx = -INFINITY;
  for (int q = 0; q < n_parts; ++q) mx = fmaxf(mx, lse_parts[q * part_rows + row]);
  float acc = 0.f, wsum = 0.f;
  for (int q = 0; q < n_parts; ++q) {
    const float l = lse_parts[q * part_rows + row];
    if (l == -INFINITY) continue;
    const float w = fast_exp2(l - mx);
    acc += w * o_parts[(q * part_rows + row) * kHeadDim + threadIdx.x];
    wsum += w;
  }
  const float v = wsum > 0.f ? acc / wsum : 0.f;
  if constexpr (sizeof(T) == 2 && std::is_same<T, __nv_bfloat16>::value)
    out[row * kHeadDim + threadIdx.x] = __float2bfloat16_rn(v);
  else
    out[row * kHeadDim + threadIdx.x] = __float2half_rn(v);
}

int launch_merge_partials(const float* o_parts, const float* lse_parts, int n_parts, long long tokens, int heads_total,
                          int heads_used, void* out, int dtype, cudaStream_t stream) {
  if (tokens == 0 || heads_used == 0) return DUO_OK;
  const unsigned grid = (unsigned)(tokens * heads_used);
  return dispatch_dtype(dtype, [&](auto t) {
    using T = decltype(t);
    merge_partials_kernel<T><<<grid, 128, 0, stream>>>(o_parts, lse_parts, n_parts, tokens, heads_total, heads_used,
                                                       (T*)out);
    DUO_CUDA_TRY(cudaGetLastError());
    return DUO_OK;
  });
}

int launch_attn_mma_partial(const duo_layer* L, long long n_keys, const void* q, long long q_row_stride, float* out_o,
                            float* out_lse, int q_len, float scale, void* workspace, size_t workspace_bytes,
                            cudaStream_t stream) {
  duo_cache_state st{};
  st.full_len = n_keys;
  st.lo = L->d.sink;
  return dispatch_dtype(L->d.dtype, [&](auto t) {
    return launch_variant<decltype(t), 4>(L, &st, q, q_row_stride, nullptr, q_len, scale, workspace, workspace_bytes,
                                          stream, {out_o, out_lse, true});
  });
}

#ifdef DUO_TRACE
extern "C" __attribute__((visibility("default"))) int duo_debug_set_trace_mma(void* buf) {
  return cudaMemcpyToSymbol(g_duo_trace_mma, &buf, sizeof(void*)) == cudaSuccess ? 0 : -3;
}
#endif

int launch_decode_fused(const duo_layer* L, const duo_cache_state* st, const void* qkv, long long row_stride,
                        const void* cos, const void* sin, int rope_mode, void* out, int q_len, float scale,
                        void* workspace, size_t workspace_bytes, cudaStream_t stream) {
  return dispatch_dtype(L->d.dtype, [&](auto t) {
    return launch_variant<decltype(t), 4, true>(L, st, qkv, row_stride, out, q_len, scale, workspace, workspace_bytes,
                                                stream, {}, {cos, sin, rope_mode});
  });
}

size_t ragged_workspace_bytes(int batch, int n_kv) { return ragged_ws_need(batch, n_kv, 2, 16); }

int launch_decode_ragged(const duo_layer* L, const long long* row_state, const long long* row_geom, const void* qkv,
                         long long row_stride, const void* cos, const void* sin, int rope_mode, void* out, int q_len,
                         float scale, void* workspace, size_t workspace_bytes, cudaStream_t stream) {
  const duo_layer_desc& d = L->d;
  duo_cache_state st{};
  st.device_state = reinterpret_cast<const int64_t*>(row_state);
  AttnParams p{};
  fill_common_params(p, d, st, qkv, row_stride, out, q_len, scale);
  fill_fused(p, d, {cos, sin, rope_mode});
  p.n_rb = 1;
  const RaggedGeom g = ragged_geom(d.batch, d.n_full, d.n_stream, sm_count_current_device(), 2, 16);
  p.rg_slots = g.slots;
  p.rg_want = g.want;
  if (d.n_full > 0)
    if (int rc = split_ws_carve(p.ws, g.ws, workspace, workspace_bytes, "duo_decode_ragged")) return rc;
  const dim3 grid(d.n_full * g.slots + d.batch * d.n_stream, 1);
  p.row_geom = row_geom;
  return dispatch_dtype(d.dtype, [&](auto t) {
    return row_geom ? launch_mma_kernel<decltype(t), 4, true, true, true>(L, grid, p, stream)
                    : launch_mma_kernel<decltype(t), 4, true, true>(L, grid, p, stream);
  });
}

int launch_decode_fused_seq(const duo_layer* L, const duo_cache_state* st, const void* qkv, long long row_stride,
                            const void* cos, const void* sin, int rope_mode, void* out, float* part_o, float* part_lse,
                            float scale, void* workspace, size_t workspace_bytes, cudaStream_t stream) {
  return dispatch_dtype(L->d.dtype, [&](auto t) {
    return launch_variant<decltype(t), 4, true>(L, st, qkv, row_stride, out, 1, scale, workspace, workspace_bytes, stream,
                                                {part_o, part_lse}, {cos, sin, rope_mode});
  });
}

int launch_attn_mma_seq(const duo_layer* L, const duo_cache_state* st, const void* q, long long q_row_stride, void* out,
                        float* part_o, float* part_lse, int q_len, float scale, void* workspace, size_t workspace_bytes,
                        cudaStream_t stream) {
  return dispatch_dtype(L->d.dtype, [&](auto t) {
    return launch_variant<decltype(t), 4>(L, st, q, q_row_stride, out, q_len, scale, workspace, workspace_bytes, stream,
                                          {part_o, part_lse});
  });
}

}
```

duo_attention_b200/csrc/duo_common.cuh:

```cuda
#pragma once
#include <cuda.h>
#include <cuda_bf16.h>
#include <cuda_fp16.h>
#include <cuda_runtime.h>
#include <stdint.h>

#include <algorithm>

#include "../../include/duo_b200.h"

namespace duo {

constexpr int kHeadDim = 128;

void set_error(const char* fmt, ...);
int cuda_fail(cudaError_t e, const char* what);
#define DUO_CUDA_TRY(expr)                                   \
  do {                                                       \
    cudaError_t _e = (expr);                                 \
    if (_e != cudaSuccess) return ::duo::cuda_fail(_e, #expr); \
  } while (0)

struct LayerMaps {
  CUtensorMap full_k64, full_v64;
  CUtensorMap ring_k64, ring_v64;
  CUtensorMap full_k128, full_v128;
  CUtensorMap ring_k128, ring_v128;
};

}

struct duo_layer {
  duo_layer_desc d;
  duo::LayerMaps maps;
  bool has_full_maps;
  bool has_ring_maps;
  int64_t pool_tokens;
};

namespace duo {

__device__ __forceinline__ uint32_t smem_u32(const void* p) {
  return static_cast<uint32_t>(__cvta_generic_to_shared(p));
}

__device__ __forceinline__ void mbar_init(uint64_t* bar, uint32_t count) {
  asm volatile("mbarrier.init.shared::cta.b64 [%0], %1;" ::"r"(smem_u32(bar)), "r"(count) : "memory");
}
__device__ __forceinline__ void mbar_expect_tx(uint64_t* bar, uint32_t bytes) {
  asm volatile("mbarrier.arrive.expect_tx.shared::cta.b64 _, [%0], %1;" ::"r"(smem_u32(bar)), "r"(bytes)
               : "memory");
}
__device__ __forceinline__ void mbar_arrive(uint64_t* bar) {
  asm volatile("mbarrier.arrive.shared::cta.b64 _, [%0];" ::"r"(smem_u32(bar)) : "memory");
}
__device__ __forceinline__ bool mbar_try_wait(uint64_t* bar, uint32_t parity) {
  uint32_t ok;
  asm volatile(
      "{\n\t.reg .pred p;\n\t"
      "mbarrier.try_wait.parity.shared::cta.b64 p, [%1], %2;\n\t"
      "selp.u32 %0, 1, 0, p;\n\t}"
      : "=r"(ok)
      : "r"(smem_u32(bar)), "r"(parity)
      : "memory");
  return ok != 0;
}
__device__ __forceinline__ void mbar_wait(uint64_t* bar, uint32_t parity) {
  uint32_t polls = 0;
  while (!mbar_try_wait(bar, parity)) {
    if (++polls == (1u << 26)) asm volatile("trap;");
  }
}
__device__ __forceinline__ void mbar_wait_spin(uint64_t* bar, uint32_t parity) {
  while (!mbar_try_wait(bar, parity)) {
  }
}
__device__ __forceinline__ void fence_barrier_init() {
  asm volatile("fence.mbarrier_init.release.cluster;" ::: "memory");
}
__device__ __forceinline__ void fence_proxy_async_smem() {
  asm volatile("fence.proxy.async.shared::cta;" ::: "memory");
}
__device__ __forceinline__ void prefetch_tmap(const CUtensorMap* m) {
  asm volatile("prefetch.tensormap [%0];" ::"l"(reinterpret_cast<uint64_t>(m)) : "memory");
}
__device__ __forceinline__ void tma_load_3d(void* smem_dst, const CUtensorMap* map, uint64_t* bar, int c0, int c1,
                                            int c2) {
  asm volatile(
      "cp.async.bulk.tensor.3d.shared::cluster.global.tile.mbarrier::complete_tx::bytes [%0], [%1, {%3, %4, %5}], "
      "[%2];" ::"r"(smem_u32(smem_dst)),
      "l"(reinterpret_cast<uint64_t>(map)), "r"(smem_u32(bar)), "r"(c0), "r"(c1), "r"(c2)
      : "memory");
}
__device__ __forceinline__ void tma_load_3d_hint(void* smem_dst, const CUtensorMap* map, uint64_t* bar, int c0, int c1,
                                                 int c2, uint64_t policy) {
  asm volatile(
      "cp.async.bulk.tensor.3d.shared::cluster.global.tile.mbarrier::complete_tx::bytes.L2::cache_hint [%0], [%1, {%3, "
      "%4, %5}], [%2], %6;" ::"r"(smem_u32(smem_dst)),
      "l"(reinterpret_cast<uint64_t>(map)), "r"(smem_u32(bar)), "r"(c0), "r"(c1), "r"(c2), "l"(policy)
      : "memory");
}
__device__ __forceinline__ uint64_t policy_evict_first() {
  uint64_t p;
  asm volatile("createpolicy.fractional.L2::evict_first.b64 %0, 1.0;" : "=l"(p));
  return p;
}
__device__ __forceinline__ uint64_t policy_evict_last() {
  uint64_t p;
  asm volatile("createpolicy.fractional.L2::evict_last.b64 %0, 1.0;" : "=l"(p));
  return p;
}

__device__ __forceinline__ void ldsm_x4(uint32_t& r0, uint32_t& r1, uint32_t& r2, uint32_t& r3, uint32_t addr) {
  asm volatile("ldmatrix.sync.aligned.m8n8.x4.shared.b16 {%0,%1,%2,%3}, [%4];"
               : "=r"(r0), "=r"(r1), "=r"(r2), "=r"(r3)
               : "r"(addr));
}
__device__ __forceinline__ void ldsm_x4_trans(uint32_t& r0, uint32_t& r1, uint32_t& r2, uint32_t& r3, uint32_t addr) {
  asm volatile("ldmatrix.sync.aligned.m8n8.x4.trans.shared.b16 {%0,%1,%2,%3}, [%4];"
               : "=r"(r0), "=r"(r1), "=r"(r2), "=r"(r3)
               : "r"(addr));
}

template <typename T>
struct MmaOp;
template <>
struct MmaOp<__nv_bfloat16> {
  __device__ __forceinline__ static void run(float (&c)[4], const uint32_t (&a)[4], uint32_t b0, uint32_t b1) {
    asm volatile(
        "mma.sync.aligned.m16n8k16.row.col.f32.bf16.bf16.f32 {%0,%1,%2,%3}, {%4,%5,%6,%7}, {%8,%9}, {%0,%1,%2,%3};"
        : "+f"(c[0]), "+f"(c[1]), "+f"(c[2]), "+f"(c[3])
        : "r"(a[0]), "r"(a[1]), "r"(a[2]), "r"(a[3]), "r"(b0), "r"(b1));
  }
  __device__ __forceinline__ static uint32_t pack(float lo, float hi) {
    __nv_bfloat162 v = __floats2bfloat162_rn(lo, hi);
    return *reinterpret_cast<uint32_t*>(&v);
  }
};
template <>
struct MmaOp<__half> {
  __device__ __forceinline__ static void run(float (&c)[4], const uint32_t (&a)[4], uint32_t b0, uint32_t b1) {
    asm volatile(
        "mma.sync.aligned.m16n8k16.row.col.f32.f16.f16.f32 {%0,%1,%2,%3}, {%4,%5,%6,%7}, {%8,%9}, {%0,%1,%2,%3};"
        : "+f"(c[0]), "+f"(c[1]), "+f"(c[2]), "+f"(c[3])
        : "r"(a[0]), "r"(a[1]), "r"(a[2]), "r"(a[3]), "r"(b0), "r"(b1));
  }
  __device__ __forceinline__ static uint32_t pack(float lo, float hi) {
    __half2 v = __floats2half2_rn(lo, hi);
    return *reinterpret_cast<uint32_t*>(&v);
  }
};

template <typename T>
struct RopeCvt;
template <>
struct RopeCvt<__nv_bfloat16> {
  __device__ static float to_f(__nv_bfloat16 v) { return __bfloat162float(v); }
  __device__ static __nv_bfloat16 from_f(float v) { return __float2bfloat16_rn(v); }
};
template <>
struct RopeCvt<__half> {
  __device__ static float to_f(__half v) { return __half2float(v); }
  __device__ static __half from_f(float v) { return __float2half_rn(v); }
};
template <typename T>
__device__ __forceinline__ float rope_hf(float x, float rot, float c, float s) {
  const float a = RopeCvt<T>::to_f(RopeCvt<T>::from_f(__fmul_rn(x, c)));
  const float r = RopeCvt<T>::to_f(RopeCvt<T>::from_f(__fmul_rn(rot, s)));
  return __fadd_rn(a, r);
}
__device__ __forceinline__ float rope_f32(float x, float rot, float c, float s) {
  return __fmaf_rn(rot, s, __fmul_rn(x, c));
}

template <typename T>
__device__ __forceinline__ void rope8(uint4& lo, uint4& hi, const void* cos, const void* sin, int mode, int tok, int d) {
  T* xl = reinterpret_cast<T*>(&lo);
  T* xh = reinterpret_cast<T*>(&hi);
#pragma unroll
  for (int e = 0; e < 8; ++e) {
    const float a = RopeCvt<T>::to_f(xl[e]), bb = RopeCvt<T>::to_f(xh[e]);
    float ol, oh;
    if (mode == DUO_ROPE_HF) {
      const T* ct = reinterpret_cast<const T*>(cos) + (long long)tok * kHeadDim;
      const T* st = reinterpret_cast<const T*>(sin) + (long long)tok * kHeadDim;
      ol = rope_hf<T>(a, -bb, RopeCvt<T>::to_f(ct[d + e]), RopeCvt<T>::to_f(st[d + e]));
      oh = rope_hf<T>(bb, a, RopeCvt<T>::to_f(ct[d + 64 + e]), RopeCvt<T>::to_f(st[d + 64 + e]));
    } else {
      const float* ct = reinterpret_cast<const float*>(cos) + (long long)tok * kHeadDim;
      const float* st = reinterpret_cast<const float*>(sin) + (long long)tok * kHeadDim;
      ol = rope_f32(a, -bb, ct[d + e], st[d + e]);
      oh = rope_f32(bb, a, ct[d + 64 + e], st[d + 64 + e]);
    }
    xl[e] = RopeCvt<T>::from_f(ol);
    xh[e] = RopeCvt<T>::from_f(oh);
  }
}

template <typename T>
struct alignas(8) Vec4 {
  T v[4];
};

__device__ __forceinline__ float warp_min(float v) {
#pragma unroll
  for (int o = 16; o > 0; o >>= 1) v = fminf(v, __shfl_xor_sync(0xffffffffu, v, o));
  return v;
}
__device__ __forceinline__ float warp_max(float v) {
#pragma unroll
  for (int o = 16; o > 0; o >>= 1) v = fmaxf(v, __shfl_xor_sync(0xffffffffu, v, o));
  return v;
}

template <typename T>
__device__ __forceinline__ void rope_row4(Vec4<T>& xv, int lane, int t, const void* cos, const void* sin, int mode) {
  Vec4<T> pv;
#pragma unroll
  for (int i = 0; i < 4; ++i) {
    const float mine = RopeCvt<T>::to_f(xv.v[i]);
    const float other = __shfl_xor_sync(0xffffffffu, mine, 16);
    pv.v[i] = RopeCvt<T>::from_f(lane < 16 ? -other : other);
  }
  if (mode == DUO_ROPE_HF) {
    const Vec4<T> cv = *reinterpret_cast<const Vec4<T>*>(reinterpret_cast<const T*>(cos) + (long long)t * kHeadDim + lane * 4);
    const Vec4<T> sv = *reinterpret_cast<const Vec4<T>*>(reinterpret_cast<const T*>(sin) + (long long)t * kHeadDim + lane * 4);
#pragma unroll
    for (int i = 0; i < 4; ++i)
      xv.v[i] = RopeCvt<T>::from_f(rope_hf<T>(RopeCvt<T>::to_f(xv.v[i]), RopeCvt<T>::to_f(pv.v[i]), RopeCvt<T>::to_f(cv.v[i]),
                                              RopeCvt<T>::to_f(sv.v[i])));
  } else {
    const float4 cv = *reinterpret_cast<const float4*>(reinterpret_cast<const float*>(cos) + (long long)t * kHeadDim + lane * 4);
    const float4 sv = *reinterpret_cast<const float4*>(reinterpret_cast<const float*>(sin) + (long long)t * kHeadDim + lane * 4);
    const float c[4] = {cv.x, cv.y, cv.z, cv.w};
    const float s[4] = {sv.x, sv.y, sv.z, sv.w};
#pragma unroll
    for (int i = 0; i < 4; ++i)
      xv.v[i] = RopeCvt<T>::from_f(rope_f32(RopeCvt<T>::to_f(xv.v[i]), RopeCvt<T>::to_f(pv.v[i]), c[i], s[i]));
  }
}

__device__ __forceinline__ void quant_row_int4(const float (&x)[4], int lane, uint8_t* packed_row, __half* scale_p,
                                               __half* zero_p) {
  float mn = fminf(fminf(x[0], x[1]), fminf(x[2], x[3]));
  float mx = fmaxf(fmaxf(x[0], x[1]), fmaxf(x[2], x[3]));
  mn = warp_min(mn);
  mx = warp_max(mx);
  const float scale = __fadd_rn(__fdiv_rn(__fsub_rn(mx, mn), 15.0f), 1e-8f);
  const float zero = mn;
  uint32_t q[4];
#pragma unroll
  for (int i = 0; i < 4; ++i) {
    float qf = __fdiv_rn(__fsub_rn(x[i], zero), scale);
    qf = roundf(qf);
    qf = fminf(fmaxf(qf, 0.0f), 15.0f);
    q[i] = (uint32_t)qf;
  }
  const uint16_t two = (uint16_t)(((q[0] << 4) | q[1]) | (((q[2] << 4) | q[3]) << 8));
  *reinterpret_cast<uint16_t*>(packed_row + 2 * lane) = two;
  if (lane == 0) {
    *scale_p = __float2half_rn(scale);
    *zero_p = __float2half_rn(zero);
  }
}

__device__ __forceinline__ void fma2(float& o0, float& o1, float a0, float a1, float b0, float b1, float c0, float c1) {
  o0 = __fmaf_rn(a0, b0, c0);
  o1 = __fmaf_rn(a1, b1, c1);
}
__device__ __forceinline__ void add2(float& o0, float& o1, float a0, float a1, float b0, float b1) {
  o0 = __fadd_rn(a0, b0);
  o1 = __fadd_rn(a1, b1);
}
__device__ __forceinline__ void mul2(float& o0, float& o1, float a0, float a1, float b0, float b1) {
  o0 = __fmul_rn(a0, b0);
  o1 = __fmul_rn(a1, b1);
}

__device__ __forceinline__ float fast_exp2(float x) {
  float y;
  asm volatile("ex2.approx.ftz.f32 %0, %1;" : "=f"(y) : "f"(x));
  return y;
}

__device__ __forceinline__ bool stream_slot_valid(int j, int sink, int recent, long long total, long long lo) {
  if (j < sink) return j < total;
  if (total <= sink) return false;
  long long last = total - 1;
  long long r = j - sink;
  long long diff = (last - sink - r) % recent;
  if (diff < 0) diff += recent;
  long long p = last - diff;
  return p >= lo;
}

template <int ROWS>
__device__ __forceinline__ void split_merge_rows4(const float* po, const float* pml, int splits, int warp, int lane,
                                                  int r0, int nr, float4 (&acc)[4], float (&mm)[4], float (&ll)[4]) {
#pragma unroll
  for (int q = 0; q < 4; ++q) {
    acc[q] = make_float4(0.f, 0.f, 0.f, 0.f);
    mm[q] = -INFINITY;
    ll[q] = 0.f;
  }
  for (int s0 = warp; s0 < splits; s0 += 16) {
    float ms[4][4], ls[4][4];
    float4 vs[4][4];
#pragma unroll
    for (int u = 0; u < 4; ++u) {
      const int s2 = s0 + 4 * u;
      const bool sok = s2 < splits;
      const int sc2 = sok ? s2 : s0;
#pragma unroll
      for (int q = 0; q < 4; ++q) {
        const bool ok = sok && q < nr;
        const int r = r0 + (q < nr ? q : 0);
        ms[u][q] = ok ? __ldcg(&pml[(sc2 * ROWS + r) * 2]) : -INFINITY;
        ls[u][q] = __ldcg(&pml[(sc2 * ROWS + r) * 2 + 1]);
        vs[u][q] = __ldcg(reinterpret_cast<const float4*>(&po[((long long)sc2 * ROWS + r) * 128 + lane * 4]));
      }
    }
#pragma unroll
    for (int u = 0; u < 4; ++u) {
#pragma unroll
      for (int q = 0; q < 4; ++q) {
        if (ms[u][q] == -INFINITY) continue;
        const float mn = fmaxf(mm[q], ms[u][q]);
        const float fo = (mm[q] == -INFINITY) ? 0.f : fast_exp2(mm[q] - mn);
        const float fn = fast_exp2(ms[u][q] - mn);
        acc[q].x = acc[q].x * fo + vs[u][q].x * fn;
        acc[q].y = acc[q].y * fo + vs[u][q].y * fn;
        acc[q].z = acc[q].z * fo + vs[u][q].z * fn;
        acc[q].w = acc[q].w * fo + vs[u][q].w * fn;
        ll[q] = ll[q] * fo + ls[u][q] * fn;
        mm[q] = mn;
      }
    }
  }
}


constexpr int kMergeGroup = 16;

struct SplitWs {
  int* counters;
  float* ws_ml;
  float* ws_o;
  float* g_ml;
  float* g_o;
  int n_groups;
};

inline int split_groups(int splits) { return splits <= kMergeGroup ? 1 : (splits + kMergeGroup - 1) / kMergeGroup; }

constexpr size_t kSplitCounterBytes = 64 * 1024;

struct SplitWsLayout {
  long long items;
  int n_groups;
  long long parts;
  long long groups;
  int rows;
};

inline SplitWsLayout split_ws_layout(long long items, int splits, int rows) {
  const int ng = split_groups(splits);
  return {items, ng, items * splits, ng > 1 ? items * ng : 0, rows};
}

inline size_t split_ws_region(long long partials, int floats_per_partial) {
  return ((size_t)partials * floats_per_partial * 4 + 255) / 256 * 256;
}

inline size_t split_ws_bytes(const SplitWsLayout& l) {
  if ((size_t)l.items * (1 + l.n_groups) * 4 > kSplitCounterBytes) return (size_t)-1;
  return kSplitCounterBytes + split_ws_region(l.parts, l.rows * 2) + split_ws_region(l.parts, l.rows * 128) +
         split_ws_region(l.groups, l.rows * 2) + split_ws_region(l.groups, l.rows * 128) + 256;
}

inline int split_ws_carve(SplitWs& w, const SplitWsLayout& l, void* workspace, size_t workspace_bytes, const char* who) {
  const size_t need = split_ws_bytes(l);
  if (need == (size_t)-1 || workspace == nullptr || workspace_bytes < need) {
    set_error("%s: workspace too small (%zu < %zu)", who, workspace_bytes, need);
    return DUO_EWORKSPACE;
  }
  uint8_t* p = reinterpret_cast<uint8_t*>(workspace);
  w.n_groups = l.n_groups;
  w.counters = reinterpret_cast<int*>(p);
  p += kSplitCounterBytes;
  w.ws_ml = reinterpret_cast<float*>(p);
  p += split_ws_region(l.parts, l.rows * 2);
  w.ws_o = reinterpret_cast<float*>(p);
  p += split_ws_region(l.parts, l.rows * 128);
  if (l.groups > 0) {
    w.g_ml = reinterpret_cast<float*>(p);
    p += split_ws_region(l.groups, l.rows * 2);
    w.g_o = reinterpret_cast<float*>(p);
  }
  return DUO_OK;
}

template <int ROWS, typename Emit>
__device__ __forceinline__ void merge_partials_cta(const float* po, const float* pml, int n, int rows, float* cm_o,
                                                   float* cm_ml, Emit emit) {
  const int tid = threadIdx.x, warp = tid >> 5, lane = tid & 31;
  for (int rg = 0; rg < rows; rg += 16) {
    const int rg_n = min(16, rows - rg);
    for (int rr0 = 0; rr0 < rg_n; rr0 += 4) {
      const int nr = min(4, rg_n - rr0);
      float4 acc4[4];
      float mm4[4], ll4[4];
      split_merge_rows4<ROWS>(po, pml, n, warp, lane, rg + rr0, nr, acc4, mm4, ll4);
#pragma unroll
      for (int q = 0; q < 4; ++q) {
        if (q < nr) {
          *reinterpret_cast<float4*>(&cm_o[(warp * 16 + rr0 + q) * 128 + lane * 4]) = acc4[q];
          if (lane == 0) {
            cm_ml[(warp * 16 + rr0 + q) * 2] = mm4[q];
            cm_ml[(warp * 16 + rr0 + q) * 2 + 1] = ll4[q];
          }
        }
      }
    }
    __syncthreads();
    for (int idx = tid; idx < rg_n * 64; idx += 128) {
      const int rr = idx >> 6, d = (idx & 63) * 2;
      float mm = -INFINITY;
#pragma unroll
      for (int w = 0; w < 4; ++w) mm = fmaxf(mm, cm_ml[(w * 16 + rr) * 2]);
      float a0f = 0.f, a1f = 0.f, ll = 0.f;
#pragma unroll
      for (int w = 0; w < 4; ++w) {
        const float mw = cm_ml[(w * 16 + rr) * 2];
        if (mw == -INFINITY) continue;
        const float f = fast_exp2(mw - mm);
        a0f += f * cm_o[(w * 16 + rr) * 128 + d];
        a1f += f * cm_o[(w * 16 + rr) * 128 + d + 1];
        ll += f * cm_ml[(w * 16 + rr) * 2 + 1];
      }
      emit(rg + rr, d, a0f, a1f, mm, ll);
    }
    __syncthreads();
  }
}

template <int ROWS, typename EmitFinal>
__device__ __forceinline__ void split_kv_finish(const SplitWs& w, long long item, int split, int splits, int rows,
                                                float* cm_o, float* cm_ml, int* s_flag, EmitFinal emit_final) {
  const int tid = threadIdx.x;
  const int ng = w.n_groups;
  int* cnt = w.counters + item * (1 + ng);
  const float* po = w.ws_o + item * splits * (long long)(ROWS * 128);
  const float* pml = w.ws_ml + item * splits * (long long)(ROWS * 2);
  auto final_emit = [&](int r, int d, float a0, float a1, float mm, float ll) {
    const float inv = ll > 0.f ? 1.f / ll : 0.f;
    emit_final(r, d, a0 * inv, a1 * inv, mm, ll);
  };
  __threadfence();
  __syncthreads();
  if (ng == 1) {
    if (tid == 0) *s_flag = (atomicAdd(&cnt[0], 1) == splits - 1);
    __syncthreads();
    if (!*s_flag) return;
    __threadfence();
    merge_partials_cta<ROWS>(po, pml, splits, rows, cm_o, cm_ml, final_emit);
    if (tid == 0) cnt[0] = 0;
    return;
  }
  const int grp = split / kMergeGroup;
  const int gsz = min(kMergeGroup, splits - grp * kMergeGroup);
  if (tid == 0) *s_flag = (atomicAdd(&cnt[1 + grp], 1) == gsz - 1);
  __syncthreads();
  if (!*s_flag) return;
  __threadfence();
  float* go = w.g_o + (item * ng + grp) * (long long)(ROWS * 128);
  float* gml = w.g_ml + (item * ng + grp) * (long long)(ROWS * 2);
  merge_partials_cta<ROWS>(po + (long long)grp * kMergeGroup * (ROWS * 128), pml + (long long)grp * kMergeGroup * (ROWS * 2),
                           gsz, rows, cm_o, cm_ml, [&](int r, int d, float a0, float a1, float mm, float ll) {
                             *reinterpret_cast<float2*>(&go[r * 128 + d]) = make_float2(a0, a1);
                             if (d == 0) {
                               gml[r * 2] = mm;
                               gml[r * 2 + 1] = ll;
                             }
                           });
  __threadfence();
  __syncthreads();
  if (tid == 0) {
    cnt[1 + grp] = 0;
    *s_flag = (atomicAdd(&cnt[0], 1) == ng - 1);
  }
  __syncthreads();
  if (!*s_flag) return;
  __threadfence();
  merge_partials_cta<ROWS>(w.g_o + item * ng * (long long)(ROWS * 128), w.g_ml + item * ng * (long long)(ROWS * 2), ng, rows,
                           cm_o, cm_ml, final_emit);
  if (tid == 0) cnt[0] = 0;
}

int sm_count_current_device();
template <typename K>
inline int ensure_dyn_smem(K kern, int bytes, unsigned long long* done_mask, bool max_carveout = false) {
  int dev = 0;
  DUO_CUDA_TRY(cudaGetDevice(&dev));
  const unsigned long long bit = 1ull << (dev & 63);
  if (__atomic_load_n(done_mask, __ATOMIC_ACQUIRE) & bit) return DUO_OK;
  DUO_CUDA_TRY(cudaFuncSetAttribute(kern, cudaFuncAttributeMaxDynamicSharedMemorySize, bytes));
  if (max_carveout)
    DUO_CUDA_TRY(cudaFuncSetAttribute(kern, cudaFuncAttributePreferredSharedMemoryCarveout, cudaSharedmemCarveoutMaxShared));
  __atomic_fetch_or(done_mask, bit, __ATOMIC_RELEASE);
  return DUO_OK;
}

__host__ __device__ __forceinline__ long long split_keys(long long nkeys, long long splits, int tile) {
  long long kps = (nkeys + splits - 1) / splits;
  kps = (kps + tile - 1) / tile * tile;
  return kps < tile ? tile : kps;
}

inline int split_want(int budget, int full_ctas, int stream_ctas) {
  const int want = (budget - stream_ctas > 0 ? budget - stream_ctas : 1) / full_ctas;
  return want < 1 ? 1 : want;
}

struct SplitPlan {
  int splits;
  long long keys_per_split;
};

inline SplitPlan plan_splits(long long nkeys, int budget, int full_ctas, int stream_ctas, int tile, int min_keys) {
  long long splits = 1;
  if (full_ctas > 0) {
    const long long max_by_len = (nkeys + min_keys - 1) / min_keys;
    splits = std::min<long long>({split_want(budget, full_ctas, stream_ctas), std::max(1LL, max_by_len), 512});
  }
  const long long kps = split_keys(nkeys, splits, tile);
  splits = (nkeys + kps - 1) / kps;
  return {(int)std::max(1LL, splits), kps};
}

__host__ __device__ __forceinline__ long long ragged_keys_per_split(long long n_sum, long long n_max, int batch,
                                                                    int want, int tile, int min_keys) {
  const long long lbar = (n_sum + batch - 1) / batch;
  long long s = (lbar + min_keys - 1) / min_keys;
  if (s < 1) s = 1;
  if (s > want) s = want;
  if (s > 512) s = 512;
  const long long kps = split_keys(lbar, s, tile);
  const long long cap = ((n_max + 511) / 512 + tile - 1) / tile * tile;
  return kps < cap ? cap : kps;
}

__device__ __forceinline__ long long ragged_batch_kps(const long long* rs, int batch, int q_add, int want, int tile,
                                                      int min_keys) {
  long long n_sum = 0, n_max = 0;
  for (int r = 0; r < batch; ++r) {
    const long long len = rs[4 * r] + q_add;
    n_sum += len;
    n_max = len > n_max ? len : n_max;
  }
  return ragged_keys_per_split(n_sum, n_max, batch, want, tile, min_keys);
}

struct RaggedSlot {
  int b, split, splits;
  long long slot_base;
};
__device__ __forceinline__ RaggedSlot ragged_slot(const long long* rs, int batch, int q_add, long long kps, int c) {
  RaggedSlot s;
  s.slot_base = 0;
  s.splits = 0;
  for (s.b = 0; s.b < batch; ++s.b) {
    const long long len = rs[4 * s.b] + q_add;
    s.splits = len > kps ? (int)((len + kps - 1) / kps) : 1;
    if (c < s.slot_base + s.splits) break;
    s.slot_base += s.splits;
  }
  s.split = c - (int)s.slot_base;
  return s;
}

template <int ROWS>
__device__ __forceinline__ void ragged_ws_slice(SplitWs& w, int b, int kvh, int n_full, int rg_slots,
                                                const RaggedSlot& s) {
  const long long item = (long long)b * n_full + kvh, ngm = w.n_groups;
  const long long part = (long long)kvh * rg_slots + s.slot_base;
  w.counters += item * (1 + ngm);
  w.ws_ml += part * (ROWS * 2);
  w.ws_o += part * (ROWS * 128);
  w.g_ml += item * ngm * (ROWS * 2);
  w.g_o += item * ngm * (ROWS * 128);
  w.n_groups = s.splits <= kMergeGroup ? 1 : (s.splits + kMergeGroup - 1) / kMergeGroup;
}

struct RaggedGeom {
  int want, slots;
  SplitWsLayout ws;
  size_t ws_bytes;
};

inline RaggedGeom ragged_geom(int batch, int n_full, int n_stream, int sm_count, int ctas_per_sm, int rows) {
  RaggedGeom g{};
  g.want = std::min(512, split_want(ctas_per_sm * sm_count, batch * std::max(n_full, 1), batch * n_stream));
  g.slots = batch * (g.want + 1);
  const long long items = (long long)batch * n_full;
  const int ng_max = split_groups(std::min(512, g.slots));
  g.ws = {items, ng_max, (long long)n_full * g.slots, items * ng_max, rows};
  g.ws_bytes = n_full > 0 ? split_ws_bytes(g.ws) : 0;
  return g;
}

inline size_t ragged_ws_need(int batch, int n_kv, int ctas_per_sm, int rows) {
  const int sms = sm_count_current_device();
  size_t need = 0;
  for (int nf = 1; nf <= n_kv; ++nf) {
    const size_t b = ragged_geom(batch, nf, n_kv - nf, sms, ctas_per_sm, rows).ws_bytes;
    if (b == (size_t)-1) return b;
    need = std::max(need, b);
  }
  return need;
}

template <typename P>
inline void fill_common_params(P& p, const duo_layer_desc& d, const duo_cache_state& st, const void* q,
                               long long q_row_stride, void* out, int q_len, float scale) {
  const int n_q = (d.n_full + d.n_stream) * d.group;
  p.q = q;
  p.out = out;
  p.q_tok_stride = q_row_stride;
  p.q_batch_stride = q_row_stride * q_len;
  p.out_batch_stride = (long long)q_len * n_q * kHeadDim;
  p.q_len = q_len;
  p.n_q_heads = n_q;
  p.group = d.group;
  p.n_full = d.n_full;
  p.n_stream = d.n_stream;
  p.batch = d.batch;
  p.sink = d.sink;
  p.recent = d.recent;
  p.W = d.sink + d.recent;
  p.full_len = st.full_len;
  p.total = st.total;
  p.lo = st.lo;
  p.dstate = reinterpret_cast<const long long*>(st.device_state);
  p.scale_log2 = scale * 1.4426950408889634f;
  p.cache_scan = (int)std::min<long long>(p.W, st.total);
}

struct FusedArgs {
  const void* cos = nullptr;
  const void* sin = nullptr;
  int rope_mode = DUO_ROPE_NONE;
};

template <typename P>
inline void fill_fused_args(P& p, const FusedArgs& fa) {
  p.cos = fa.cos;
  p.sin = fa.sin;
  p.rope_mode = fa.rope_mode;
  p.k_off = (long long)p.n_q_heads * kHeadDim;
  p.v_off = (long long)(p.n_q_heads + p.n_full + p.n_stream) * kHeadDim;
}

struct KvMaps {
  const CUtensorMap *fk, *fv, *rk, *rv;
};
inline KvMaps kv_maps(const duo_layer* L, bool box128) {
  const LayerMaps& m = L->maps;
  const CUtensorMap* fk = box128 ? &m.full_k128 : &m.full_k64;
  const CUtensorMap* fv = box128 ? &m.full_v128 : &m.full_v64;
  const CUtensorMap* rk = box128 ? &m.ring_k128 : &m.ring_k64;
  const CUtensorMap* rv = box128 ? &m.ring_v128 : &m.ring_v64;
  return {L->has_full_maps ? fk : rk, L->has_full_maps ? fv : rv, L->has_ring_maps ? rk : fk,
          L->has_ring_maps ? rv : fv};
}

template <typename F>
inline int dispatch_dtype(int dtype, F&& f) {
  if (dtype == DUO_DT_BF16) return f(__nv_bfloat16{});
  return f(__half{});
}

}
```

duo_attention_b200/csrc/elementwise.cu:

```cuda
#include "duo_common.cuh"

namespace duo {

template <typename T>
struct EwCvt;
template <>
struct EwCvt<__nv_bfloat16> {
  __device__ static float to_f(__nv_bfloat16 v) { return __bfloat162float(v); }
  __device__ static __nv_bfloat16 from_f(float v) { return __float2bfloat16_rn(v); }
};
template <>
struct EwCvt<__half> {
  __device__ static float to_f(__half v) { return __half2float(v); }
  __device__ static __half from_f(float v) { return __float2half_rn(v); }
};

template <typename T>
struct alignas(16) Vec8 {
  T v[8];
};

template <typename T>
__global__ void __launch_bounds__(256) add_rmsnorm_kernel(const T* __restrict__ x, const T* __restrict__ residual,
                                                          const T* __restrict__ weight, T* __restrict__ out_norm,
                                                          T* __restrict__ out_res, int hidden, float eps) {
  extern __shared__ float s_row[];
  __shared__ float s_part[8];
  const long long row = blockIdx.x;
  const T* xr = x + row * hidden;
  const T* rr = residual ? residual + row * hidden : nullptr;
  float ss = 0.f;
  for (int i = threadIdx.x * 8; i < hidden; i += blockDim.x * 8) {
    Vec8<T> a = *reinterpret_cast<const Vec8<T>*>(xr + i);
    if (rr) {
      const Vec8<T> b = *reinterpret_cast<const Vec8<T>*>(rr + i);
#pragma unroll
      for (int k = 0; k < 8; ++k) a.v[k] = EwCvt<T>::from_f(EwCvt<T>::to_f(b.v[k]) + EwCvt<T>::to_f(a.v[k]));
      if (out_res) *reinterpret_cast<Vec8<T>*>(out_res + row * hidden + i) = a;
    }
#pragma unroll
    for (int k = 0; k < 8; ++k) {
      const float f = EwCvt<T>::to_f(a.v[k]);
      s_row[i + k] = f;
      ss += f * f;
    }
  }
#pragma unroll
  for (int o = 16; o > 0; o >>= 1) ss += __shfl_xor_sync(0xffffffffu, ss, o);
  if ((threadIdx.x & 31) == 0) s_part[threadIdx.x >> 5] = ss;
  __syncthreads();
  float tot = 0.f;
#pragma unroll
  for (int w = 0; w < 8; ++w) tot += (w < (int)(blockDim.x >> 5)) ? s_part[w] : 0.f;
  const float inv = rsqrtf(tot / (float)hidden + eps);
  for (int i = threadIdx.x * 8; i < hidden; i += blockDim.x * 8) {
    const Vec8<T> w = *reinterpret_cast<const Vec8<T>*>(weight + i);
    Vec8<T> o;
#pragma unroll
    for (int k = 0; k < 8; ++k) {
      const T n = EwCvt<T>::from_f(s_row[i + k] * inv);
      o.v[k] = EwCvt<T>::from_f(EwCvt<T>::to_f(w.v[k]) * EwCvt<T>::to_f(n));
    }
    *reinterpret_cast<Vec8<T>*>(out_norm + row * hidden + i) = o;
  }
}

template <typename T>
__global__ void __launch_bounds__(256) silu_mul_kernel(const T* __restrict__ gate_up, T* __restrict__ out, long long rows,
                                                       int inter) {
  const long long per_row = inter / 8;
  const long long idx = (long long)blockIdx.x * blockDim.x + threadIdx.x;
  if (idx >= rows * per_row) return;
  const long long row = idx / per_row;
  const int c = (int)(idx % per_row) * 8;
  const Vec8<T> g = *reinterpret_cast<const Vec8<T>*>(gate_up + row * 2 * inter + c);
  const Vec8<T> u = *reinterpret_cast<const Vec8<T>*>(gate_up + row * 2 * inter + inter + c);
  Vec8<T> o;
#pragma unroll
  for (int k = 0; k < 8; ++k) {
    const float gf = EwCvt<T>::to_f(g.v[k]);
    const T act = EwCvt<T>::from_f(gf / (1.0f + __expf(-gf)));
    o.v[k] = EwCvt<T>::from_f(EwCvt<T>::to_f(act) * EwCvt<T>::to_f(u.v[k]));
  }
  *reinterpret_cast<Vec8<T>*>(out + row * inter + c) = o;
}

int launch_add_rmsnorm(const void* x, const void* residual, const void* weight, void* out_norm, void* out_res,
                       long long rows, int hidden, float eps, int dtype, cudaStream_t stream) {
  if (rows == 0) return DUO_OK;
  const size_t smem = (size_t)hidden * sizeof(float);
  if (smem > 48 * 1024) {
    static unsigned long long mask_bf = 0, mask_h = 0;
    const int rc = dtype == DUO_DT_BF16 ? ensure_dyn_smem(add_rmsnorm_kernel<__nv_bfloat16>, 64 * 1024, &mask_bf)
                                        : ensure_dyn_smem(add_rmsnorm_kernel<__half>, 64 * 1024, &mask_h);
    if (rc) return rc;
  }
  if (dtype == DUO_DT_BF16) {
    add_rmsnorm_kernel<__nv_bfloat16><<<(unsigned)rows, 256, smem, stream>>>(
        (const __nv_bfloat16*)x, (const __nv_bfloat16*)residual, (const __nv_bfloat16*)weight, (__nv_bfloat16*)out_norm,
        (__nv_bfloat16*)out_res, hidden, eps);
  } else {
    add_rmsnorm_kernel<__half><<<(unsigned)rows, 256, smem, stream>>>((const __half*)x, (const __half*)residual,
                                                                      (const __half*)weight, (__half*)out_norm,
                                                                      (__half*)out_res, hidden, eps);
  }
  DUO_CUDA_TRY(cudaGetLastError());
  return DUO_OK;
}

int launch_silu_mul(const void* gate_up, void* out, long long rows, int inter, int dtype, cudaStream_t stream) {
  if (rows == 0) return DUO_OK;
  const long long n = rows * (inter / 8);
  const unsigned blocks = (unsigned)((n + 255) / 256);
  if (dtype == DUO_DT_BF16)
    silu_mul_kernel<__nv_bfloat16><<<blocks, 256, 0, stream>>>((const __nv_bfloat16*)gate_up, (__nv_bfloat16*)out, rows, inter);
  else
    silu_mul_kernel<__half><<<blocks, 256, 0, stream>>>((const __half*)gate_up, (__half*)out, rows, inter);
  DUO_CUDA_TRY(cudaGetLastError());
  return DUO_OK;
}

}
```

duo_attention_b200/ops.py:

```python
from __future__ import annotations

import torch

from . import _C

LAUNCHES = 0


def _dt(t):
    if t.dtype == torch.bfloat16:
        return _C.DT_BF16
    if t.dtype == torch.float16:
        return _C.DT_FP16
    raise ValueError(f"dtype {t.dtype} not supported (bf16 / fp16)")


def add_rmsnorm(x: torch.Tensor, residual, weight: torch.Tensor, eps: float, inplace_residual: bool = True):
    global LAUNCHES
    if not x.is_cuda:
        raise RuntimeError("duo_attention_b200 kernels need CUDA tensors (no CPU fallback)")
    hidden = x.shape[-1]
    x = x if x.is_contiguous() else x.contiguous()
    rows = x.numel() // hidden
    out = torch.empty_like(x)
    res_ptr, out_res, h = None, None, x
    if residual is not None:
        assert residual.is_contiguous() and residual.shape == x.shape and residual.dtype == x.dtype
        h = residual if inplace_residual else torch.empty_like(x)
        res_ptr, out_res = residual.data_ptr(), h.data_ptr()
    _C.check(_C.load().duo_add_rmsnorm(x.data_ptr(), res_ptr, weight.data_ptr(), out.data_ptr(), out_res, rows, hidden,
                                      float(eps), _dt(x), torch.cuda.current_stream(x.device).cuda_stream))
    LAUNCHES += 1
    return out, h


def silu_mul(gate_up: torch.Tensor):
    global LAUNCHES
    if not gate_up.is_cuda:
        raise RuntimeError("duo_attention_b200 kernels need CUDA tensors (no CPU fallback)")
    inter = gate_up.shape[-1] // 2
    gate_up = gate_up if gate_up.is_contiguous() else gate_up.contiguous()
    rows = gate_up.numel() // (2 * inter)
    out = torch.empty(*gate_up.shape[:-1], inter, dtype=gate_up.dtype, device=gate_up.device)
    _C.check(_C.load().duo_silu_mul(gate_up.data_ptr(), out.data_ptr(), rows, inter, _dt(gate_up),
                                   torch.cuda.current_stream(gate_up.device).cuda_stream))
    LAUNCHES += 1
    return out
```

duo_attention_b200/patch/hf_driver.py:

```python
from __future__ import annotations

import types
from typing import Optional

import torch
from transformers.modeling_outputs import CausalLMOutputWithPast

from .. import _C
from ..kv_cache import DuoKVCache, DuoRaggedKVCache, model_geometry


class _AttnPlan:

    def __init__(self, n_full, n_kv, group, head_dim):
        self.n_full, self.n_kv, self.group, self.head_dim = n_full, n_kv, group, head_dim
        self.wqkv = None
        self.bqkv = None


def _fuse_qkv(attn):
    plan = attn._duo_plan
    w = torch.cat([attn.q_proj.weight.data, attn.k_proj.weight.data, attn.v_proj.weight.data], dim=0).contiguous()
    nq, nk = attn.q_proj.weight.shape[0], attn.k_proj.weight.shape[0]
    attn.q_proj.weight.data = w[:nq]
    attn.k_proj.weight.data = w[nq : nq + nk]
    attn.v_proj.weight.data = w[nq + nk :]
    plan.wqkv = w
    if attn.q_proj.bias is not None:
        plan.bqkv = torch.cat([attn.q_proj.bias.data, attn.k_proj.bias.data, attn.v_proj.bias.data]).contiguous()


def _fuse_gate_up(mlp):
    w = torch.cat([mlp.gate_proj.weight.data, mlp.up_proj.weight.data], dim=0).contiguous()
    n = mlp.gate_proj.weight.shape[0]
    mlp.gate_proj.weight.data = w[:n]
    mlp.up_proj.weight.data = w[n:]
    mlp._duo_wgu = w


def _mlp_forward(mlp, x):
    from .. import ops

    w = getattr(mlp, "_duo_wgu", None)
    if w is None or w.device != x.device:
        _fuse_gate_up(mlp)
        w = mlp._duo_wgu
    return mlp.down_proj(ops.silu_mul(torch.nn.functional.linear(x, w)))


def _fusable(layer):
    m = layer.mlp
    return (all(hasattr(m, n) for n in ("gate_proj", "up_proj", "down_proj"))
            and m.gate_proj.bias is None and m.up_proj.bias is None
            and type(getattr(m, "act_fn", None)).__name__ in ("SiLU", "SiLUActivation")
            and hasattr(layer.input_layernorm, "variance_epsilon"))


def duo_attention_layer_forward(attn, hidden_states, cos, sin, kv_cache: DuoKVCache, layer_idx: int,
                                rope_mode: int = _C.ROPE_HF, project: bool = True):
    plan = attn._duo_plan
    if plan.wqkv is None or plan.wqkv.device != hidden_states.device:
        _fuse_qkv(attn)
    B, S, _ = hidden_states.shape
    qkv = torch.nn.functional.linear(hidden_states, plan.wqkv, plan.bqkv)
    out = torch.empty(B, S, plan.n_kv * plan.group, plan.head_dim, dtype=qkv.dtype, device=qkv.device)
    kv_cache.attend(layer_idx, qkv, cos, sin, rope_mode, out)
    return attn.o_proj(out.view(B, S, -1)) if project else out.view(B, S, -1)


def _tp_layer_pipelined(layer, ctx, h, next_norm, group, n_blocks):
    import torch.distributed as dist

    from .. import ops

    S = ctx.shape[1]
    step = (S + n_blocks - 1) // n_blocks
    spans = [(r, min(S, r + step)) for r in range(0, S, step)]
    ln2 = layer.post_attention_layernorm
    parts, works = [], []
    for r0, r1 in spans:
        a = layer.self_attn.o_proj(ctx[:, r0:r1])
        works.append(dist.all_reduce(a, op=dist.ReduceOp.SUM, group=group, async_op=True))
        parts.append(a)
    mparts, mworks = [], []
    for (r0, r1), a, w in zip(spans, parts, works):
        w.wait()
        x, _ = ops.add_rmsnorm(a, h[:, r0:r1], ln2.weight, ln2.variance_epsilon)
        m = _mlp_forward(layer.mlp, x)
        mworks.append(dist.all_reduce(m, op=dist.ReduceOp.SUM, group=group, async_op=True))
        mparts.append(m)
    outs = []
    for (r0, r1), m, w in zip(spans, mparts, mworks):
        w.wait()
        x, _ = ops.add_rmsnorm(m, h[:, r0:r1], next_norm.weight, next_norm.variance_epsilon)
        outs.append(x)
    return torch.cat(outs, dim=1)


def plans_head_dim(model):
    return model.model.layers[0].self_attn._duo_plan.head_dim


def _rope_theta_and_scale(cfg):
    rp = getattr(cfg, "rope_parameters", None) or {}
    rs = getattr(cfg, "rope_scaling", None) or {}
    theta = getattr(cfg, "rope_theta", None) or rp.get("rope_theta") or 10000.0
    factor = rs.get("factor") or rp.get("factor") or 1.0
    return float(theta), float(factor)


def _new_dynamic_cache(model, batch_size, first_len):
    plans = [layer.self_attn._duo_plan for layer in model.model.layers]
    p = next(model.parameters())
    cfg = model.config
    return DuoKVCache(
        num_layers=len(plans),
        num_heads=cfg.num_attention_heads,
        num_kv_heads=cfg.num_key_value_heads,
        head_dim=plans[0].head_dim,
        num_full_kv_head_list=[pl.n_full for pl in plans],
        batch_size=batch_size,
        max_size=max(256, 2 * first_len),
        sink_size=model._duo_sink,
        recent_size=model._duo_recent,
        dtype=p.dtype,
        device=p.device,
        stage_cap=first_len,
        growable=True,
    )


def duo_causal_lm_forward(self, input_ids: Optional[torch.LongTensor] = None, attention_mask=None,
                          position_ids=None, past_key_values=None, inputs_embeds=None, labels=None,
                          use_cache=None, **kwargs):
    if labels is not None:
        raise ValueError("the DuoAttention eval forward does not compute a loss")
    base = self.model
    if inputs_embeds is None:
        inputs_embeds = base.embed_tokens(input_ids)
    B, S, _ = inputs_embeds.shape
    cache = past_key_values
    if cache is None:
        cache = _new_dynamic_cache(self, B, S)
    elif not isinstance(cache, DuoKVCache):
        raise ValueError("past_key_values must be None or a DuoKVCache produced by this model")
    ragged = isinstance(cache, DuoRaggedKVCache)
    if ragged:
        if S * cache.num_kv_groups > cache.max_rows:
            raise ValueError(f"a DuoRaggedKVCache takes decode-sized chunks (group x q_len <= {cache.max_rows}, got "
                             f"{S} tokens): prefill each row through cache.row(b)")
        if getattr(self, "_duo_tp", False) or getattr(self, "_duo_seq", None) is not None:
            raise ValueError("DuoRaggedKVCache is not supported with tensor-parallel or sequence-sharded models")
        if position_ids is None:
            first = torch.tensor(cache.row_lengths, dtype=torch.long, device=inputs_embeds.device)
            position_ids = first[:, None] + torch.arange(S, dtype=torch.long, device=inputs_embeds.device)[None]
        else:
            position_ids = position_ids.view(B, S).long()
    else:
        past_len = cache.kv_seq_len
        if position_ids is None:
            position_ids = torch.arange(past_len, past_len + S, dtype=torch.long, device=inputs_embeds.device)[None]
        else:
            position_ids = position_ids.view(-1, S).long()[:1]
    rope_mode = getattr(self, "_duo_rope_mode", _C.ROPE_HF)
    if ragged and rope_mode == _C.ROPE_FP32:
        theta, factor = _rope_theta_and_scale(self.config)
        pos = position_ids.to(torch.float32) / factor
        idx = torch.arange(plans_head_dim(self) // 2, dtype=torch.float32, device=pos.device)
        ang = pos[..., None] * torch.pow(torch.tensor(theta, device=pos.device), -2.0 * idx / plans_head_dim(self))
        cos, sin = torch.cat([ang.cos(), ang.cos()], -1).contiguous(), torch.cat([ang.sin(), ang.sin()], -1).contiguous()
    elif ragged:
        cos, sin = base.rotary_emb(inputs_embeds, position_ids)
        cos, sin = cos.contiguous(), sin.contiguous()
    elif rope_mode == _C.ROPE_FP32:
        theta, factor = _rope_theta_and_scale(self.config)
        pos = position_ids[0].to(torch.float32) / factor
        idx = torch.arange(plans_head_dim(self) // 2, dtype=torch.float32, device=pos.device)
        ang = pos[:, None] * torch.pow(torch.tensor(theta, device=pos.device), -2.0 * idx / plans_head_dim(self))[None]
        cos, sin = torch.cat([ang.cos(), ang.cos()], -1).contiguous(), torch.cat([ang.sin(), ang.sin()], -1).contiguous()
    else:
        cos, sin = base.rotary_emb(inputs_embeds, position_ids)
        cos, sin = cos[0].contiguous(), sin[0].contiguous()
    h = inputs_embeds.contiguous() if input_ids is not None else inputs_embeds.clone()
    tp_on = getattr(self, "_duo_tp", False)
    seq_on = getattr(self, "_duo_seq", None) is not None
    if tp_on:
        from ..tp import all_reduce_sum
    layers = list(base.layers)
    if h.is_cuda and h.shape[-1] % 8 == 0 and all(_fusable(l) for l in layers):
        from .. import ops

        comm = getattr(self, "_duo_comm", None) if tp_on else None
        if comm is not None and not comm.usable(h):
            comm = None

        def reduce_add_norm(part, res, w, eps):
            if comm is not None:
                return comm.add_rmsnorm(part, res, w, eps)
            if tp_on:
                part = all_reduce_sum(part, self._duo_tp_group)
            return ops.add_rmsnorm(part, res, w, eps)

        x, _ = ops.add_rmsnorm(h, None, layers[0].input_layernorm.weight, layers[0].input_layernorm.variance_epsilon)
        pipe_rows = getattr(self, "_duo_tp_pipeline_rows", 4096)
        pipelined = tp_on and not seq_on and comm is None and B == 1 and S >= pipe_rows
        for idx, layer in enumerate(layers):
            if pipelined and idx + 1 < len(layers):
                ctx = duo_attention_layer_forward(layer.self_attn, x, cos, sin, cache, idx, rope_mode, project=False)
                x = _tp_layer_pipelined(layer, ctx, h, layers[idx + 1].input_layernorm, self._duo_tp_group,
                                        getattr(self, "_duo_tp_pipeline_blocks", 2))
                continue
            a = duo_attention_layer_forward(layer.self_attn, x, cos, sin, cache, idx, rope_mode)
            ln2 = layer.post_attention_layernorm
            if seq_on:
                x, h = ops.add_rmsnorm(a, h, ln2.weight, ln2.variance_epsilon)
            else:
                x, h = reduce_add_norm(a, h, ln2.weight, ln2.variance_epsilon)
            m = _mlp_forward(layer.mlp, x)
            if idx + 1 < len(layers):
                nxt = layers[idx + 1].input_layernorm
                x, h = reduce_add_norm(m, h, nxt.weight, nxt.variance_epsilon)
            else:
                if tp_on and comm is None:
                    m = all_reduce_sum(m, self._duo_tp_group)
                m_last, h_last = m[:, -1:, :].contiguous(), h[:, -1:, :].contiguous()
                if comm is not None:
                    x, _ = comm.add_rmsnorm(m_last, h_last, base.norm.weight, base.norm.variance_epsilon)
                else:
                    x, _ = ops.add_rmsnorm(m_last, h_last, base.norm.weight, base.norm.variance_epsilon)
        h = x
    else:
        for idx, layer in enumerate(layers):
            res = h
            x = layer.input_layernorm(h)
            x = duo_attention_layer_forward(layer.self_attn, x, cos, sin, cache, idx, rope_mode)
            if tp_on and not seq_on:
                x = all_reduce_sum(x, self._duo_tp_group)
            h = res + x
            res = h
            x = layer.post_attention_layernorm(h)
            x = layer.mlp(x)
            if tp_on:
                x = all_reduce_sum(x, self._duo_tp_group)
            h = res + x
        h = base.norm(h[:, -1:, :])
    if cache.dev_state is not None:
        cache.advance_device(S)
    logits = self.lm_head(h)
    if getattr(self, "_duo_logits_float", True):
        logits = logits.float()
    return CausalLMOutputWithPast(logits=logits, past_key_values=cache if use_cache is not False else None)


def install(model, full_attention_heads, sink_size, recent_size, logits_float=True, rope="hf"):
    from .reorder import reorder_linear_weights, reorder_full_attn_heads

    geo = model_geometry(model)
    n_kv, head_dim = geo["num_kv_heads"], geo["head_dim"]
    group = geo["num_heads"] // n_kv
    for idx, layer in enumerate(model.model.layers):
        module = layer.self_attn
        gate = torch.tensor(full_attention_heads[idx], device=geo["device"], dtype=geo["dtype"])
        reorder_linear_weights(module.q_proj, gate, group * head_dim, "out")
        reorder_linear_weights(module.k_proj, gate, head_dim, "out")
        reorder_linear_weights(module.v_proj, gate, head_dim, "out")
        reorder_linear_weights(module.o_proj, gate, group * head_dim, "in")
        gate = reorder_full_attn_heads(gate)
        module.sink_size = sink_size
        module.recent_size = recent_size
        module.register_buffer("full_attention_heads", gate)
        module._duo_plan = _AttnPlan(int((gate > 0.5).sum().item()), n_kv, group, head_dim)
    model._duo_sink = sink_size
    model._duo_recent = recent_size
    model._duo_logits_float = logits_float
    if rope not in ("hf", "flashinfer"):
        raise ValueError(f"rope must be 'hf' or 'flashinfer', got {rope!r}")
    model._duo_rope_mode = _C.ROPE_FP32 if rope == "flashinfer" else _C.ROPE_HF
    model.forward = types.MethodType(duo_causal_lm_forward, model)
    return model
```

include/duo_b200.h:

```cpp
#ifndef DUO_B200_H
#define DUO_B200_H

#include <stddef.h>
#include <stdint.h>

#ifdef __cplusplus
extern "C" {
#endif

#if defined(__GNUC__)
#define DUO_API __attribute__((visibility("default")))
#else
#define DUO_API
#endif

#define DUO_OK 0
#define DUO_EINVAL -1
#define DUO_EOVERFLOW -2
#define DUO_ECUDA -3
#define DUO_EWORKSPACE -4

#define DUO_DT_BF16 0
#define DUO_DT_FP16 1
#define DUO_KV_SAME 0
#define DUO_KV_INT4 1

#define DUO_ROPE_NONE 0
#define DUO_ROPE_HF 1
#define DUO_ROPE_FP32 2
#define DUO_ROPE_SKIP_Q 0x100

typedef struct duo_layer_desc {
  void* full_k;
  void* full_v;
  void* ring_k;
  void* ring_v;
  void* full_k_scale;
  void* full_k_zero;
  void* full_v_scale;
  void* full_v_zero;
  void* ring_k_scale;
  void* ring_k_zero;
  void* ring_v_scale;
  void* ring_v_zero;
  int64_t full_cap;
  int32_t batch;
  int32_t n_full;
  int32_t n_stream;
  int32_t group;
  int32_t head_dim;
  int32_t sink;
  int32_t recent;
  int32_t stage_cap;
  int32_t dtype;
  int32_t kv_format;
} duo_layer_desc;

typedef struct duo_cache_state {
  int64_t full_len;
  int64_t total;
  int64_t lo;
  const int64_t* device_state;
  int32_t seq_rank, seq_world, seq_block, seq_reserved;
} duo_cache_state;

typedef struct duo_layer duo_layer;

DUO_API int duo_layer_create(const duo_layer_desc* desc, duo_layer** out);
DUO_API void duo_layer_destroy(duo_layer* layer);

DUO_API size_t duo_workspace_bytes(int32_t batch, int32_t n_kv_heads, int32_t group, int32_t max_q_len);

DUO_API int duo_rope_append(const duo_layer* layer, const duo_cache_state* st, void* qkv, int64_t qkv_row_stride,
                    const void* cos, const void* sin, int32_t rope_mode, int32_t q_len, void* stream);

#define DUO_DECODE_MAX_Q 16
DUO_API int duo_attention(const duo_layer* layer, const duo_cache_state* st, const void* q, int64_t q_row_stride,
                  void* out, int32_t q_len, float scale, void* workspace, size_t workspace_bytes,
                  void* stream);

#define DUO_DECODE_MAX_Q_INT4 8
DUO_API int duo_decode_fused(const duo_layer* layer, const duo_cache_state* st, const void* qkv, int64_t qkv_row_stride,
                             const void* cos, const void* sin, int32_t rope_mode, void* out, int32_t q_len, float scale,
                             void* workspace, size_t workspace_bytes, void* stream);

#define DUO_RAGGED_MAX_BATCH 64
DUO_API int duo_decode_ragged(const duo_layer* layer, const int64_t* row_state, int64_t max_full_len, const void* qkv,
                              int64_t qkv_row_stride, const void* cos, const void* sin, int32_t rope_mode, void* out,
                              int32_t q_len, float scale, void* workspace, size_t workspace_bytes, void* stream);
DUO_API size_t duo_ragged_workspace_bytes(int32_t batch, int32_t n_kv_heads);
DUO_API int duo_decode_ragged_int4(const duo_layer* layer, const int64_t* row_state, int64_t max_full_len,
                                   const void* qkv, int64_t qkv_row_stride, const void* cos, const void* sin,
                                   int32_t rope_mode, void* out, int32_t q_len, float scale, void* workspace,
                                   size_t workspace_bytes, void* stream);
DUO_API size_t duo_ragged_int4_workspace_bytes(int32_t batch, int32_t n_kv_heads);
DUO_API int duo_layer_create_pooled(const duo_layer_desc* desc, int64_t pool_tokens, duo_layer** out);
DUO_API int duo_decode_ragged_pooled(const duo_layer* layer, const int64_t* row_state, const int64_t* row_geom,
                                     int64_t min_room, const void* qkv, int64_t qkv_row_stride, const void* cos,
                                     const void* sin, int32_t rope_mode, void* out, int32_t q_len, float scale,
                                     void* workspace, size_t workspace_bytes, void* stream);
DUO_API int duo_ragged_state_advance(int64_t* row_state, int32_t batch, int32_t n, int32_t sink, int32_t recent,
                                     void* stream);

DUO_API int duo_attention_mma(const duo_layer* layer, const duo_cache_state* st, const void* q, int64_t q_row_stride,
                              void* out, int32_t q_len, float scale, void* workspace, size_t workspace_bytes,
                              void* stream);

DUO_API int duo_state_advance(int64_t* device_state, int32_t n, int32_t sink, int32_t recent, void* stream);
DUO_API int duo_state_set(int64_t* device_state, int64_t full_len, int64_t total, int64_t lo, void* stream);

DUO_API int duo_stream_commit(const duo_layer* layer, const duo_cache_state* st, int32_t q_len, void* stream);

DUO_API int duo_quant_int4(const void* in, int64_t in_row_stride, int64_t rows, void* packed, void* scale,
                   void* zero, void* stream);
DUO_API int duo_dequant_int4(const void* packed, const void* scale, const void* zero, int64_t rows, void* out,
                     void* stream);
DUO_API int duo_dequant_int4_bf16(const void* packed, const void* scale, const void* zero, int64_t rows, void* out,
                                  void* stream);

DUO_API int duo_add_rmsnorm(const void* x, const void* residual, const void* weight, void* out_norm, void* out_res,
                            int64_t rows, int32_t hidden, float eps, int32_t dtype, void* stream);
DUO_API int duo_silu_mul(const void* gate_up, void* out, int64_t rows, int32_t inter, int32_t dtype, void* stream);

DUO_API int duo_attention_partial(const duo_layer* layer, int64_t n_keys, const void* q, int64_t q_row_stride,
                                  float* out_o, float* out_lse, int32_t q_len, float scale, void* workspace,
                                  size_t workspace_bytes, void* stream);
DUO_API int duo_attention_seq(const duo_layer* layer, const duo_cache_state* st, const void* q, int64_t q_row_stride,
                              void* out, float* out_o, float* out_lse, int32_t q_len, float scale, void* workspace,
                              size_t workspace_bytes, void* stream);
DUO_API int duo_decode_fused_seq(const duo_layer* layer, const duo_cache_state* st, const void* qkv, int64_t qkv_row_stride,
                                 const void* cos, const void* sin, int32_t rope_mode, void* out, float* out_o,
                                 float* out_lse, float scale, void* workspace, size_t workspace_bytes, void* stream);
DUO_API int duo_merge_partials(const float* o_parts, const float* lse_parts, int32_t n_parts, int64_t tokens,
                               int32_t heads_total, int32_t heads_used, void* out, int32_t dtype, void* stream);

typedef struct duo_comm duo_comm;
typedef struct duo_comm_desc {
  void* data[8];
  void* flags[8];
  void* local_state;
  int32_t rank, world;
  int32_t hidden;
  int32_t max_rows;
  int32_t dtype;
} duo_comm_desc;
DUO_API size_t duo_comm_data_bytes(int32_t world, int32_t hidden, int32_t max_rows, int32_t dtype);
DUO_API size_t duo_comm_flag_bytes(int32_t world, int32_t max_rows);
DUO_API int duo_comm_create(const duo_comm_desc* desc, duo_comm** out);
DUO_API void duo_comm_destroy(duo_comm* comm);
DUO_API int duo_allreduce_add_rmsnorm(const duo_comm* comm, const void* partial, const void* residual,
                                      const void* weight, void* out_norm, void* out_res, int32_t rows, float eps,
                                      void* stream);

typedef struct duo_seqcomm duo_seqcomm;
typedef struct duo_seqcomm_desc {
  void* data[8];
  void* flags[8];
  void* local_state;
  int32_t rank, world;
  int32_t max_rows;
} duo_seqcomm_desc;
DUO_API size_t duo_seqcomm_data_bytes(int32_t world, int32_t max_rows);
DUO_API size_t duo_seqcomm_flag_bytes(int32_t world, int32_t max_rows);
DUO_API int duo_seqcomm_create(const duo_seqcomm_desc* desc, duo_seqcomm** out);
DUO_API void duo_seqcomm_destroy(duo_seqcomm* comm);
DUO_API int duo_seq_merge(const duo_seqcomm* comm, const float* part_o, const float* part_lse, void* out, int32_t tokens,
                          int32_t heads_total, int32_t heads_used, int32_t dtype, void* stream);

DUO_API const char* duo_last_error_string(void);
DUO_API int duo_version(void);

#ifdef __cplusplus
}
#endif
#endif
```

Measured before the change: 56.47.

## Add fused TMA-pipelined decode GEMV with norm/SiLU epilogues and PDL chaining

Adds a persistent GEMV kernel for small-M decode that uses a producer warp issuing bulk async copies with an evict-first L2 hint into a 16-stage mbarrier ring. Consumer warps compute the product with an optional fused add+RMSNorm prologue and SiLU-mul or fp32 epilogue. The decode forward path calls it for the qkv, o_proj, gate_up, down and lm_head projections. Programmatic dependent launch is added to the fused decode attention kernel and the GEMV so that consecutive kernels overlap their launch and prologue. The goal is to move weight reads closer to DRAM bandwidth and remove separate norm and activation kernels, at the cost of a large custom code path and possible numerical differences.

```diff
diff --git a/duo_attention_b200/_C.py b/duo_attention_b200/_C.py
--- a/duo_attention_b200/_C.py
+++ b/duo_attention_b200/_C.py
@@ -14,13 +14,16 @@
 DECODE_MAX_Q = 16
 DECODE_MAX_Q_INT4 = 8
 RAGGED_MAX_BATCH = 64
+GEMV_SILU, GEMV_NORM, GEMV_F32_OUT = 1, 2, 4
+GEMV_MAX_M = 8
+GEMV_NORM_MAX_ELEMS = 32768
 
 SYMBOLS = [
     "duo_layer_create", "duo_layer_destroy", "duo_workspace_bytes", "duo_rope_append", "duo_attention",
     "duo_attention_mma", "duo_decode_fused", "duo_decode_ragged", "duo_ragged_workspace_bytes",
     "duo_decode_ragged_int4", "duo_ragged_int4_workspace_bytes", "duo_layer_create_pooled", "duo_decode_ragged_pooled",
     "duo_ragged_state_advance", "duo_state_advance", "duo_state_set", "duo_stream_commit", "duo_quant_int4", "duo_dequant_int4", "duo_dequant_int4_bf16", "duo_add_rmsnorm", "duo_silu_mul",
-    "duo_attention_partial", "duo_merge_partials", "duo_attention_seq", "duo_decode_fused_seq",
+    "duo_gemv", "duo_gemv_plan", "duo_attention_partial", "duo_merge_partials", "duo_attention_seq", "duo_decode_fused_seq",
     "duo_seqcomm_data_bytes", "duo_seqcomm_flag_bytes", "duo_seqcomm_create", "duo_seqcomm_destroy", "duo_seq_merge",
     "duo_comm_data_bytes", "duo_comm_flag_bytes", "duo_comm_create", "duo_comm_destroy", "duo_allreduce_add_rmsnorm",
     "duo_last_error_string", "duo_version",
@@ -114,6 +117,10 @@
     lib.duo_add_rmsnorm.restype = C.c_int
     lib.duo_silu_mul.argtypes = [vp, vp, i64, i32, i32, vp]
     lib.duo_silu_mul.restype = C.c_int
+    lib.duo_gemv.argtypes = [vp, vp, vp, vp, f32, vp, vp, vp, i32, i32, i32, i32, i32, vp]
+    lib.duo_gemv.restype = C.c_int
+    lib.duo_gemv_plan.argtypes = [i32, i32, i32, i32, i32, C.POINTER(i32)]
+    lib.duo_gemv_plan.restype = C.c_int
     lib.duo_attention_partial.argtypes = [vp, i64, vp, i64, vp, vp, i32, f32, vp, sz, vp]
     lib.duo_attention_partial.restype = C.c_int
     lib.duo_attention_seq.argtypes = [vp, C.POINTER(CacheState), vp, i64, vp, vp, vp, i32, f32, vp, sz, vp]
diff --git a/duo_attention_b200/csrc/api.cu b/duo_attention_b200/csrc/api.cu
--- a/duo_attention_b200/csrc/api.cu
+++ b/duo_attention_b200/csrc/api.cu
@@ -84,6 +84,9 @@
 int launch_add_rmsnorm(const void* x, const void* residual, const void* weight, void* out_norm, void* out_res,
                        long long rows, int hidden, float eps, int dtype, cudaStream_t stream);
 int launch_silu_mul(const void* gate_up, void* out, long long rows, int inter, int dtype, cudaStream_t stream);
+int launch_gemv(const void* x, const void* residual, const void* norm_weight, void* out_res, float eps, const void* w,
+                const void* bias, void* y, int m, int n, int k, int flags, int dtype, cudaStream_t stream);
+int gemv_plan_host(int m, int n, int k, int flags, int sms, int* out);
 
 typedef CUresult (*EncodeTiledFn)(CUtensorMap*, CUtensorMapDataType, cuuint32_t, void*, const cuuint64_t*,
                                   const cuuint64_t*, const cuuint32_t*, const cuuint32_t*, CUtensorMapInterleave,
@@ -609,6 +612,26 @@
   return launch_silu_mul(gate_up, out, rows, inter, dtype, (cudaStream_t)stream);
 }
 
+int duo_gemv(const void* x, const void* residual, const void* norm_weight, void* out_res, float eps, const void* w,
+             const void* bias, void* y, int32_t m, int32_t n, int32_t k, int32_t flags, int32_t dtype, void* stream) {
+  const uintptr_t align = (uintptr_t)x | (uintptr_t)w | (uintptr_t)residual | (uintptr_t)norm_weight |
+                          (uintptr_t)out_res;
+  if (!x || !w || !y || ((flags & DUO_GEMV_NORM) && !norm_weight) || (align & 15) != 0 ||
+      (dtype != DUO_DT_BF16 && dtype != DUO_DT_FP16)) {
+    set_error("duo_gemv: bad argument");
+    return DUO_EINVAL;
+  }
+  return launch_gemv(x, residual, norm_weight, out_res, eps, w, bias, y, m, n, k, flags, dtype, (cudaStream_t)stream);
+}
+
+int duo_gemv_plan(int32_t m, int32_t n, int32_t k, int32_t flags, int32_t sm_count, int32_t* out) {
+  if (!out || gemv_plan_host(m, n, k, flags, sm_count, out) != DUO_OK) {
+    set_error("duo_gemv_plan: unsupported shape m=%d n=%d k=%d flags=%d", m, n, k, flags);
+    return DUO_EINVAL;
+  }
+  return DUO_OK;
+}
+
 int duo_dequant_int4(const void* packed, const void* scale, const void* zero, int64_t rows, void* out, void* stream) {
   if (rows < 0 || (rows > 0 && (!packed || !scale || !zero || !out))) {
     set_error("duo_dequant_int4: bad argument");
diff --git a/duo_attention_b200/csrc/attn_mma.cu b/duo_attention_b200/csrc/attn_mma.cu
--- a/duo_attention_b200/csrc/attn_mma.cu
+++ b/duo_attention_b200/csrc/attn_mma.cu
@@ -98,6 +98,7 @@
   static_assert(!RAGGED || (FUSED && KEY_WARPS == 4), "the ragged variant is the fused decode kernel");
   static_assert(!POOLED || RAGGED, "the pooled layout is a ragged decode layout");
   DUO_TRACE_MMA(0);
+  if constexpr (FUSED && KEY_WARPS == 4) pdl_wait();
   AttnParams p = pin;
   if (!RAGGED && pin.dstate) {
     p.full_len = pin.dstate[0];
@@ -458,6 +459,7 @@
   }
 
   __syncthreads();
+  if constexpr (FUSED && KEY_WARPS == 4) pdl_launch_dependents();
   float* sm_o = reinterpret_cast<float*>(smem);
   float* sm_ml = reinterpret_cast<float*>(smem + 64 * 1024);
   if constexpr (KEY_WARPS == 4) {
@@ -597,6 +599,8 @@
   static unsigned long long attr_mask = 0;
   if (int rc = ensure_dyn_smem(kern, ATTN_SMEM_BYTES, &attr_mask)) return rc;
   const KvMaps m = kv_maps(L, false);
+  if constexpr (FUSED && KEY_WARPS == 4)
+    return launch_pdl(kern, grid, dim3(ATTN_THREADS), ATTN_SMEM_BYTES, stream, *m.fk, *m.fv, *m.rk, *m.rv, p);
   kern<<<grid, ATTN_THREADS, ATTN_SMEM_BYTES, stream>>>(*m.fk, *m.fv, *m.rk, *m.rv, p);
   DUO_CUDA_TRY(cudaGetLastError());
   return DUO_OK;
diff --git a/duo_attention_b200/csrc/duo_common.cuh b/duo_attention_b200/csrc/duo_common.cuh
--- a/duo_attention_b200/csrc/duo_common.cuh
+++ b/duo_attention_b200/csrc/duo_common.cuh
@@ -6,6 +6,7 @@
 #include <stdint.h>
 
 #include <algorithm>
+#include <utility>
 
 #include "../../include/duo_b200.h"
 
@@ -194,6 +195,97 @@
     }
     xl[e] = RopeCvt<T>::from_f(ol);
     xh[e] = RopeCvt<T>::from_f(oh);
+  }
+}
+
+__device__ __forceinline__ void pdl_wait() { asm volatile("griddepcontrol.wait;" ::: "memory"); }
+__device__ __forceinline__ void pdl_launch_dependents() { asm volatile("griddepcontrol.launch_dependents;" ::: "memory"); }
+
+__device__ __forceinline__ void bulk_load_hint(void* smem_dst, const void* src, uint32_t bytes, uint64_t* bar,
+                                               uint64_t policy) {
+  asm volatile(
+      "cp.async.bulk.shared::cluster.global.mbarrier::complete_tx::bytes.L2::cache_hint [%0], [%1], %2, [%3], %4;" ::"r"(
+          smem_u32(smem_dst)),
+      "l"(reinterpret_cast<uint64_t>(src)), "r"(bytes), "r"(smem_u32(bar)), "l"(policy)
+      : "memory");
+}
+
+__device__ __forceinline__ void named_bar_sync(int id, int threads) {
+  asm volatile("bar.sync %0, %1;" ::"r"(id), "r"(threads) : "memory");
+}
+
+template <typename... KArgs, typename... Args>
+inline int launch_pdl(void (*kern)(KArgs...), dim3 grid, dim3 block, size_t smem, cudaStream_t stream, Args&&... args) {
+  cudaLaunchConfig_t cfg = {};
+  cfg.gridDim = grid;
+  cfg.blockDim = block;
+  cfg.dynamicSmemBytes = smem;
+  cfg.stream = stream;
+  cudaLaunchAttribute attr[1];
+  attr[0].id = cudaLaunchAttributeProgrammaticStreamSerialization;
+  attr[0].val.programmaticStreamSerializationAllowed = 1;
+  cfg.attrs = attr;
+  cfg.numAttrs = 1;
+  DUO_CUDA_TRY(cudaLaunchKernelEx(&cfg, kern, std::forward<Args>(args)...));
+  return DUO_OK;
+}
+
+template <typename T>
+struct EwCvt;
+template <>
+struct EwCvt<__nv_bfloat16> {
+  __device__ static float to_f(__nv_bfloat16 v) { return __bfloat162float(v); }
+  __device__ static __nv_bfloat16 from_f(float v) { return __float2bfloat16_rn(v); }
+};
+template <>
+struct EwCvt<__half> {
+  __device__ static float to_f(__half v) { return __half2float(v); }
+  __device__ static __half from_f(float v) { return __float2half_rn(v); }
+};
+
+template <typename T>
+struct alignas(16) Vec8 {
+  T v[8];
+};
+
+template <typename T, typename Sync>
+__device__ __forceinline__ void add_rmsnorm_row(const T* __restrict__ xr, const T* __restrict__ rr,
+                                                const T* __restrict__ weight, T* out_norm, T* __restrict__ out_res,
+                                                int hidden, float eps, float* s_row, float* s_part, int tid,
+                                                int nthreads, Sync sync) {
+  float ss = 0.f;
+  for (int i = tid * 8; i < hidden; i += nthreads * 8) {
+    Vec8<T> a = *reinterpret_cast<const Vec8<T>*>(xr + i);
+    if (rr) {
+      const Vec8<T> b = *reinterpret_cast<const Vec8<T>*>(rr + i);
+#pragma unroll
+      for (int k = 0; k < 8; ++k) a.v[k] = EwCvt<T>::from_f(EwCvt<T>::to_f(b.v[k]) + EwCvt<T>::to_f(a.v[k]));
+      if (out_res) *reinterpret_cast<Vec8<T>*>(out_res + i) = a;
+    }
+#pragma unroll
+    for (int k = 0; k < 8; ++k) {
+      const float f = EwCvt<T>::to_f(a.v[k]);
+      s_row[i + k] = f;
+      ss += f * f;
+    }
+  }
+#pragma unroll
+  for (int o = 16; o > 0; o >>= 1) ss += __shfl_xor_sync(0xffffffffu, ss, o);
+  if ((tid & 31) == 0) s_part[tid >> 5] = ss;
+  sync();
+  float tot = 0.f;
+#pragma unroll
+  for (int w = 0; w < 8; ++w) tot += (w < (nthreads >> 5)) ? s_part[w] : 0.f;
+  const float inv = rsqrtf(tot / (float)hidden + eps);
+  for (int i = tid * 8; i < hidden; i += nthreads * 8) {
+    const Vec8<T> w = *reinterpret_cast<const Vec8<T>*>(weight + i);
+    Vec8<T> o;
+#pragma unroll
+    for (int k = 0; k < 8; ++k) {
+      const T n = EwCvt<T>::from_f(s_row[i + k] * inv);
+      o.v[k] = EwCvt<T>::from_f(EwCvt<T>::to_f(w.v[k]) * EwCvt<T>::to_f(n));
+    }
+    *reinterpret_cast<Vec8<T>*>(out_norm + i) = o;
   }
 }
 
diff --git a/duo_attention_b200/csrc/elementwise.cu b/duo_attention_b200/csrc/elementwise.cu
--- a/duo_attention_b200/csrc/elementwise.cu
+++ b/duo_attention_b200/csrc/elementwise.cu
@@ -1,24 +1,6 @@
 #include "duo_common.cuh"
 
 namespace duo {
-
-template <typename T>
-struct EwCvt;
-template <>
-struct EwCvt<__nv_bfloat16> {
-  __device__ static float to_f(__nv_bfloat16 v) { return __bfloat162float(v); }
-  __device__ static __nv_bfloat16 from_f(float v) { return __float2bfloat16_rn(v); }
-};
-template <>
-struct EwCvt<__half> {
-  __device__ static float to_f(__half v) { return __half2float(v); }
-  __device__ static __half from_f(float v) { return __float2half_rn(v); }
-};
-
-template <typename T>
-struct alignas(16) Vec8 {
-  T v[8];
-};
 
 template <typename T>
 __global__ void __launch_bounds__(256) add_rmsnorm_kernel(const T* __restrict__ x, const T* __restrict__ residual,
@@ -27,42 +9,9 @@
   extern __shared__ float s_row[];
   __shared__ float s_part[8];
   const long long row = blockIdx.x;
-  const T* xr = x + row * hidden;
-  const T* rr = residual ? residual + row * hidden : nullptr;
-  float ss = 0.f;
-  for (int i = threadIdx.x * 8; i < hidden; i += blockDim.x * 8) {
-    Vec8<T> a = *reinterpret_cast<const Vec8<T>*>(xr + i);
-    if (rr) {
-      const Vec8<T> b = *reinterpret_cast<const Vec8<T>*>(rr + i);
-#pragma unroll
-      for (int k = 0; k < 8; ++k) a.v[k] = EwCvt<T>::from_f(EwCvt<T>::to_f(b.v[k]) + EwCvt<T>::to_f(a.v[k]));
-      if (out_res) *reinterpret_cast<Vec8<T>*>(out_res + row * hidden + i) = a;
-    }
-#pragma unroll
-    for (int k = 0; k < 8; ++k) {
-      const float f = EwCvt<T>::to_f(a.v[k]);
-      s_row[i + k] = f;
-      ss += f * f;
-    }
-  }
-#pragma unroll
-  for (int o = 16; o > 0; o >>= 1) ss += __shfl_xor_sync(0xffffffffu, ss, o);
-  if ((threadIdx.x & 31) == 0) s_part[threadIdx.x >> 5] = ss;
-  __syncthreads();
-  float tot = 0.f;
-#pragma unroll
-  for (int w = 0; w < 8; ++w) tot += (w < (int)(blockDim.x >> 5)) ? s_part[w] : 0.f;
-  const float inv = rsqrtf(tot / (float)hidden + eps);
-  for (int i = threadIdx.x * 8; i < hidden; i += blockDim.x * 8) {
-    const Vec8<T> w = *reinterpret_cast<const Vec8<T>*>(weight + i);
-    Vec8<T> o;
-#pragma unroll
-    for (int k = 0; k < 8; ++k) {
-      const T n = EwCvt<T>::from_f(s_row[i + k] * inv);
-      o.v[k] = EwCvt<T>::from_f(EwCvt<T>::to_f(w.v[k]) * EwCvt<T>::to_f(n));
-    }
-    *reinterpret_cast<Vec8<T>*>(out_norm + row * hidden + i) = o;
-  }
+  add_rmsnorm_row<T>(x + row * hidden, residual ? residual + row * hidden : nullptr, weight, out_norm + row * hidden,
+                     out_res ? out_res + row * hidden : nullptr, hidden, eps, s_row, s_part, threadIdx.x, blockDim.x,
+                     [] { __syncthreads(); });
 }
 
 template <typename T>
diff --git a/duo_attention_b200/csrc/gemv.cu b/duo_attention_b200/csrc/gemv.cu
--- /dev/null
+++ b/duo_attention_b200/csrc/gemv.cu
@@ -0,0 +1,315 @@
+#include "duo_common.cuh"
+
+namespace duo {
+
+constexpr int GV_ROWS = 16;
+constexpr int GV_KC = 256;
+constexpr int GV_STAGES = 16;
+constexpr int GV_PITCH = GV_KC * 2 + 16;
+constexpr int GV_STAGE_BYTES = GV_ROWS * GV_PITCH;
+constexpr int GV_WARPS = 8;
+constexpr int GV_CONSUMERS = GV_WARPS * 32;
+constexpr int GV_THREADS = GV_CONSUMERS + 32;
+constexpr int GV_X_ELEMS = 32768;
+constexpr int GV_SMEM_MAX = 226 * 1024;
+constexpr int GV_BAR = 1;
+constexpr int GV_SPLIT_MAX_N = 4096;
+
+struct GemvParams {
+  const void* w;
+  const void* bias;
+  const void* x;
+  const void* res;
+  const void* norm_w;
+  void* out_res;
+  void* y;
+  float eps;
+  int m, n, k;
+  int ks, nslices;
+  int kps, splits;
+  int tiles;
+  int inter;
+};
+
+struct GemvPlan {
+  int tiles, grid, ks, nslices, kps, splits, smem;
+};
+
+inline GemvPlan gemv_plan(int m, int n, int k, int flags, int sms) {
+  GemvPlan pl{};
+  pl.tiles = (flags & DUO_GEMV_SILU) ? (n / 2 + 7) / 8 : (n + GV_ROWS - 1) / GV_ROWS;
+  pl.grid = std::min(sms, pl.tiles);
+  const int per = GV_X_ELEMS / m;
+  pl.ks = per >= k ? k : per / GV_KC * GV_KC;
+  pl.nslices = (k + pl.ks - 1) / pl.ks;
+  pl.splits = (n <= GV_SPLIT_MAX_N && k >= 128) ? 2 : 1;
+  pl.kps = pl.splits == 2 ? (k / 64 + 1) / 2 * 64 : k;
+  pl.smem = GV_STAGES * GV_STAGE_BYTES + m * (pl.ks * 2 + 16) + 16 + ((flags & DUO_GEMV_NORM) ? k * 4 : 0);
+  return pl;
+}
+
+enum : int { GV_EPI_PLAIN = 0, GV_EPI_SILU = 1, GV_EPI_F32 = 2 };
+
+template <typename F>
+__device__ __forceinline__ void for_each_segment(const GemvParams& p, F&& f) {
+  for (int s = 0; s < p.nslices; ++s) {
+    const int k_lo = s * p.ks, k_hi = min(p.k, k_lo + p.ks);
+    for (int sp = 0; sp < p.splits; ++sp) {
+      const int a = max(k_lo, sp * p.kps), b = min(k_hi, sp + 1 == p.splits ? p.k : (sp + 1) * p.kps);
+      if (a < b) f(a, b, sp, s);
+    }
+  }
+}
+
+template <typename T, bool NORM, int EPI>
+__global__ void __launch_bounds__(GV_THREADS, 1) duo_gemv_kernel(const GemvParams p) {
+  using Cv = EwCvt<T>;
+  extern __shared__ __align__(128) uint8_t gv_smem[];
+  __shared__ __align__(8) uint64_t full_bar[GV_STAGES];
+  __shared__ __align__(8) uint64_t empty_bar[GV_STAGES];
+  __shared__ float s_part[8];
+
+  const int tid = threadIdx.x, warp = tid >> 5, lane = tid & 31;
+  const int xpitch = p.ks * 2 + 16;
+  uint8_t* ring = gv_smem;
+  uint8_t* xs = ring + GV_STAGES * GV_STAGE_BYTES;
+  uint8_t* zero16 = xs + p.m * xpitch;
+  float* s_row = reinterpret_cast<float*>(zero16 + 16);
+  const int t0 = (int)((long long)blockIdx.x * p.tiles / gridDim.x);
+  const int t1 = (int)((long long)(blockIdx.x + 1) * p.tiles / gridDim.x);
+
+  if (tid == 0) {
+    for (int s = 0; s < GV_STAGES; ++s) {
+      mbar_init(&full_bar[s], 1);
+      mbar_init(&empty_bar[s], 1);
+    }
+    fence_barrier_init();
+  }
+  if (tid < 4) reinterpret_cast<uint32_t*>(zero16)[tid] = 0u;
+  __syncthreads();
+
+  if (warp == GV_WARPS) {
+    const T* W = reinterpret_cast<const T*>(p.w);
+    const uint64_t pol = policy_evict_first();
+    int uses[GV_STAGES] = {};
+    for (int r0 = t0; r0 < t1; r0 += GV_WARPS) {
+      const int nw = min(GV_WARPS, t1 - r0), spw = GV_STAGES / nw;
+      int q = 0;
+      for_each_segment(p, [&](int a, int b, int, int) {
+        for (int k0 = a; k0 < b; k0 += GV_KC, ++q) {
+          const int bytes = min(GV_KC, b - k0) * 2;
+          for (int w = 0; w < nw; ++w) {
+            const int t = r0 + w;
+            long long row = -1;
+            if (EPI == GV_EPI_SILU) {
+              const int i = 8 * t + (lane & 7);
+              if (lane < GV_ROWS && i < p.inter) row = lane < 8 ? i : p.inter + i;
+            } else {
+              const long long r = (long long)GV_ROWS * t + lane;
+              if (lane < GV_ROWS && r < p.n) row = r;
+            }
+            const unsigned live = __ballot_sync(0xffffffffu, row >= 0);
+            const int st = w + nw * (q % spw);
+            const int u = uses[st]++;
+            if (u > 0) mbar_wait(&empty_bar[st], (u - 1) & 1);
+            if (lane == 0) mbar_expect_tx(&full_bar[st], (uint32_t)(__popc(live) * bytes));
+            __syncwarp();
+            if (row >= 0)
+              bulk_load_hint(ring + st * GV_STAGE_BYTES + lane * GV_PITCH, W + row * p.k + k0, (uint32_t)bytes,
+                             &full_bar[st], pol);
+          }
+        }
+      });
+    }
+    pdl_launch_dependents();
+    pdl_wait();
+    return;
+  }
+
+  pdl_wait();
+  using Op = MmaOp<T>;
+  const T* X = reinterpret_cast<const T*>(p.x);
+  const int g = lane >> 2, t4 = lane & 3;
+  const int a_row = (lane & 7) + ((lane >> 3) & 1) * 8, a_col = (lane >> 4) * 8;
+  const uint32_t a_base = smem_u32(ring) + a_row * GV_PITCH + a_col * 2;
+  const int b_tok = lane & 7;
+  const bool b_live = b_tok < p.m;
+  const uint32_t b_base = b_live ? smem_u32(xs) + b_tok * xpitch + (lane >> 3) * 8 * 2 : smem_u32(zero16);
+  const uint32_t b_elem = b_live ? 2u : 0u;
+
+  auto load_x = [&](int k_lo, int k_hi) {
+    named_bar_sync(GV_BAR, GV_CONSUMERS);
+    if constexpr (NORM) {
+      const T* R = reinterpret_cast<const T*>(p.res);
+      T* out_res = (blockIdx.x == 0 && R) ? reinterpret_cast<T*>(p.out_res) : nullptr;
+      for (int r = 0; r < p.m; ++r) {
+        add_rmsnorm_row<T>(X + (long long)r * p.k, R ? R + (long long)r * p.k : nullptr,
+                           reinterpret_cast<const T*>(p.norm_w), reinterpret_cast<T*>(xs + r * xpitch),
+                           out_res ? out_res + (long long)r * p.k : nullptr, p.k, p.eps, s_row, s_part, tid,
+                           GV_CONSUMERS, [] { named_bar_sync(GV_BAR, GV_CONSUMERS); });
+        named_bar_sync(GV_BAR, GV_CONSUMERS);
+      }
+    } else {
+      const int vpr = (k_hi - k_lo) / 8;
+      for (int i = tid; i < p.m * vpr; i += GV_CONSUMERS) {
+        const int r = i / vpr, c = (i - r * vpr) * 8;
+        *reinterpret_cast<uint4*>(xs + r * xpitch + c * 2) =
+            *reinterpret_cast<const uint4*>(X + (long long)r * p.k + k_lo + c);
+      }
+      named_bar_sync(GV_BAR, GV_CONSUMERS);
+    }
+  };
+  if (p.nslices == 1) load_x(0, p.k);
+
+  int uses[GV_STAGES] = {};
+  for (int r0 = t0; r0 < t1; r0 += GV_WARPS) {
+    const int nw = min(GV_WARPS, t1 - r0), spw = GV_STAGES / nw;
+    const bool mine = warp < nw;
+    int q = 0;
+    const int t = r0 + warp;
+    float c[4] = {0.f, 0.f, 0.f, 0.f}, tot[4] = {0.f, 0.f, 0.f, 0.f};
+    for_each_segment(p, [&](int a, int b, int sp, int s) {
+      const int k_lo = s * p.ks;
+      if (p.nslices > 1 && a == k_lo) load_x(k_lo, min(p.k, k_lo + p.ks));
+      if (sp > 0 && a == sp * p.kps) {
+#pragma unroll
+        for (int e = 0; e < 4; ++e) {
+          tot[e] = sp == 1 ? c[e] : tot[e] + c[e];
+          c[e] = 0.f;
+        }
+      }
+      for (int k0 = a; k0 < b; k0 += GV_KC, ++q) {
+        const int st0 = nw * (q % spw);
+        const int u = uses[st0 + (mine ? warp : 0)];
+        for (int w = 0; w < nw; ++w) ++uses[st0 + w];
+        if (!mine) continue;
+        const int st = st0 + warp;
+        mbar_wait(&full_bar[st], u & 1);
+        const int steps = min(GV_KC, b - k0) / 32;
+        const uint32_t as = a_base + st * GV_STAGE_BYTES;
+        const uint32_t bs = b_base + (uint32_t)(k0 - k_lo) * b_elem;
+        uint32_t bf[GV_KC / 32][4], a0[GV_KC / 32][4], a1[GV_KC / 32][4];
+#pragma unroll
+        for (int j = 0; j < GV_KC / 32; ++j) {
+          if (j < steps) {
+            ldsm_x4(bf[j][0], bf[j][1], bf[j][2], bf[j][3], bs + j * 32 * b_elem);
+            ldsm_x4(a0[j][0], a0[j][1], a0[j][2], a0[j][3], as + j * 64);
+            ldsm_x4(a1[j][0], a1[j][1], a1[j][2], a1[j][3], as + j * 64 + 32);
+          }
+        }
+#pragma unroll
+        for (int j = 0; j < GV_KC / 32; ++j) {
+          if (j < steps) {
+            Op::run(c, a0[j], bf[j][0], bf[j][1]);
+            Op::run(c, a1[j], bf[j][2], bf[j][3]);
+          }
+        }
+        __syncwarp();
+        if (lane == 0) mbar_arrive(&empty_bar[st]);
+      }
+    });
+    named_bar_sync(GV_BAR, GV_CONSUMERS);
+    if (!mine) continue;
+    if (p.splits > 1) {
+#pragma unroll
+      for (int e = 0; e < 4; ++e) c[e] = tot[e] + c[e];
+    }
+    if (EPI == GV_EPI_SILU) {
+      const int i = 8 * t + g;
+#pragma unroll
+      for (int e = 0; e < 2; ++e) {
+        const int n = 2 * t4 + e;
+        if (n < p.m && i < p.inter) {
+          const T gt = Cv::from_f(c[e]), ut = Cv::from_f(c[e + 2]);
+          const float gf = Cv::to_f(gt);
+          const T act = Cv::from_f(gf / (1.0f + __expf(-gf)));
+          reinterpret_cast<T*>(p.y)[(long long)n * p.inter + i] = Cv::from_f(Cv::to_f(act) * Cv::to_f(ut));
+        }
+      }
+    } else {
+#pragma unroll
+      for (int e = 0; e < 4; ++e) {
+        const int n = 2 * t4 + (e & 1);
+        const long long row = (long long)GV_ROWS * t + g + 8 * (e >> 1);
+        if (n < p.m && row < p.n) {
+          float v = c[e];
+          if (p.bias) v += Cv::to_f(reinterpret_cast<const T*>(p.bias)[row]);
+          if (EPI == GV_EPI_F32)
+            reinterpret_cast<float*>(p.y)[(long long)n * p.n + row] = Cv::to_f(Cv::from_f(v));
+          else
+            reinterpret_cast<T*>(p.y)[(long long)n * p.n + row] = Cv::from_f(v);
+        }
+      }
+    }
+  }
+}
+
+template <typename T, bool NORM, int EPI>
+static int launch_gemv_t(const GemvParams& p, const GemvPlan& pl, cudaStream_t stream) {
+  auto kern = duo_gemv_kernel<T, NORM, EPI>;
+  static unsigned long long attr_mask = 0;
+  if (int rc = ensure_dyn_smem(kern, GV_SMEM_MAX, &attr_mask)) return rc;
+  return launch_pdl(kern, dim3(pl.grid), dim3(GV_THREADS), (size_t)pl.smem, stream, p);
+}
+
+template <typename T, bool NORM>
+static int launch_gemv_epi(const GemvParams& p, const GemvPlan& pl, int flags, cudaStream_t stream) {
+  if (flags & DUO_GEMV_SILU) return launch_gemv_t<T, NORM, GV_EPI_SILU>(p, pl, stream);
+  if (flags & DUO_GEMV_F32_OUT) return launch_gemv_t<T, NORM, GV_EPI_F32>(p, pl, stream);
+  return launch_gemv_t<T, NORM, GV_EPI_PLAIN>(p, pl, stream);
+}
+
+int gemv_check(int m, int n, int k, int flags, int sms, GemvPlan* out) {
+  if (m < 1 || m > DUO_GEMV_MAX_M || n < 1 || k < 64 || k % 64 != 0 || (flags & ~7) != 0 ||
+      ((flags & DUO_GEMV_SILU) && ((flags & DUO_GEMV_F32_OUT) || n % 2 != 0)) || sms < 1)
+    return DUO_EINVAL;
+  const GemvPlan pl = gemv_plan(m, n, k, flags, sms);
+  if (((flags & DUO_GEMV_NORM) && pl.nslices != 1) || pl.smem > GV_SMEM_MAX) return DUO_EINVAL;
+  if (out) *out = pl;
+  return DUO_OK;
+}
+
+int gemv_plan_host(int m, int n, int k, int flags, int sms, int* out) {
+  GemvPlan pl{};
+  if (int rc = gemv_check(m, n, k, flags, sms, &pl)) return rc;
+  out[0] = pl.grid;
+  out[1] = pl.tiles;
+  out[2] = pl.ks;
+  out[3] = pl.smem;
+  return DUO_OK;
+}
+
+int launch_gemv(const void* x, const void* residual, const void* norm_weight, void* out_res, float eps, const void* w,
+                const void* bias, void* y, int m, int n, int k, int flags, int dtype, cudaStream_t stream) {
+  GemvPlan pl{};
+  if (gemv_check(m, n, k, flags, sm_count_current_device(), &pl) != DUO_OK) {
+    set_error("duo_gemv: unsupported shape m=%d n=%d k=%d flags=%d (m <= %d, k %% 64 == 0, NORM: m*k <= %d)", m, n, k,
+              flags, DUO_GEMV_MAX_M, GV_X_ELEMS);
+    return DUO_EINVAL;
+  }
+  GemvParams p{};
+  p.w = w;
+  p.bias = bias;
+  p.x = x;
+  p.res = residual;
+  p.norm_w = norm_weight;
+  p.out_res = out_res;
+  p.y = y;
+  p.eps = eps;
+  p.m = m;
+  p.n = n;
+  p.k = k;
+  p.ks = pl.ks;
+  p.nslices = pl.nslices;
+  p.tiles = pl.tiles;
+  p.kps = pl.kps;
+  p.splits = pl.splits;
+  p.inter = n / 2;
+  const bool norm = flags & DUO_GEMV_NORM;
+  return dispatch_dtype(dtype, [&](auto t) {
+    using T = decltype(t);
+    return norm ? launch_gemv_epi<T, true>(p, pl, flags, stream) : launch_gemv_epi<T, false>(p, pl, flags, stream);
+  });
+}
+
+}
diff --git a/duo_attention_b200/ops.py b/duo_attention_b200/ops.py
--- a/duo_attention_b200/ops.py
+++ b/duo_attention_b200/ops.py
@@ -34,6 +34,46 @@
     return out, h
 
 
+def gemv(x: torch.Tensor, w: torch.Tensor, bias=None, *, residual=None, norm_weight=None, eps: float = 0.0,
+         silu: bool = False, out_float: bool = False):
+    global LAUNCHES
+    if not x.is_cuda:
+        raise RuntimeError("duo_attention_b200 kernels need CUDA tensors (no CPU fallback)")
+    K = x.shape[-1]
+    N = w.shape[0]
+    assert w.is_contiguous() and w.shape[1] == K and w.dtype == x.dtype
+    x = x if x.is_contiguous() else x.contiguous()
+    m = x.numel() // K
+    flags = (_C.GEMV_SILU if silu else 0) | (_C.GEMV_F32_OUT if out_float else 0)
+    n_out = N // 2 if silu else N
+    y = torch.empty(*x.shape[:-1], n_out, dtype=torch.float32 if out_float else x.dtype, device=x.device)
+    res_ptr = out_res = nor_ptr = None
+    h = None
+    if norm_weight is not None:
+        flags |= _C.GEMV_NORM
+        nor_ptr = norm_weight.data_ptr()
+        h = x
+        if residual is not None:
+            assert residual.is_contiguous() and residual.shape == x.shape and residual.dtype == x.dtype
+            h = torch.empty_like(x)
+            res_ptr, out_res = residual.data_ptr(), h.data_ptr()
+    if bias is not None:
+        assert bias.is_contiguous() and bias.numel() == N and bias.dtype == x.dtype
+    _C.check(_C.load().duo_gemv(x.data_ptr(), res_ptr, nor_ptr, out_res, float(eps), w.data_ptr(),
+                                bias.data_ptr() if bias is not None else None, y.data_ptr(), m, N, K, flags, _dt(x),
+                                torch.cuda.current_stream(x.device).cuda_stream))
+    LAUNCHES += 1
+    return y if norm_weight is None else (y, h)
+
+
+def gemv_plan(m: int, n: int, k: int, flags: int, sm_count: int):
+    import ctypes
+
+    out = (ctypes.c_int32 * 4)()
+    _C.check(_C.load().duo_gemv_plan(m, n, k, flags, sm_count, out))
+    return dict(grid=out[0], tiles=out[1], k_slice=out[2], smem=out[3])
+
+
 def silu_mul(gate_up: torch.Tensor):
     global LAUNCHES
     if not gate_up.is_cuda:
diff --git a/duo_attention_b200/patch/hf_driver.py b/duo_attention_b200/patch/hf_driver.py
--- a/duo_attention_b200/patch/hf_driver.py
+++ b/duo_attention_b200/patch/hf_driver.py
@@ -58,14 +58,67 @@
 
 def duo_attention_layer_forward(attn, hidden_states, cos, sin, kv_cache: DuoKVCache, layer_idx: int,
                                 rope_mode: int = _C.ROPE_HF, project: bool = True):
+    qkv = torch.nn.functional.linear(hidden_states, *_qkv_weights(attn, hidden_states.device))
+    out = _attend(attn, qkv, cos, sin, kv_cache, layer_idx, rope_mode)
+    return attn.o_proj(out) if project else out
+
+
+def _qkv_weights(attn, device):
     plan = attn._duo_plan
-    if plan.wqkv is None or plan.wqkv.device != hidden_states.device:
+    if plan.wqkv is None or plan.wqkv.device != device:
         _fuse_qkv(attn)
-    B, S, _ = hidden_states.shape
-    qkv = torch.nn.functional.linear(hidden_states, plan.wqkv, plan.bqkv)
+    return plan.wqkv, plan.bqkv
+
+
+def _attend(attn, qkv, cos, sin, kv_cache, layer_idx, rope_mode):
+    plan = attn._duo_plan
+    B, S, _ = qkv.shape
     out = torch.empty(B, S, plan.n_kv * plan.group, plan.head_dim, dtype=qkv.dtype, device=qkv.device)
     kv_cache.attend(layer_idx, qkv, cos, sin, rope_mode, out)
-    return attn.o_proj(out.view(B, S, -1)) if project else out.view(B, S, -1)
+    return out.view(B, S, -1)
+
+
+DECODE_GEMV_ROWS = 1
+
+
+def decode_gemv_eligible(model, h) -> bool:
+    B, S, hidden = h.shape
+    rows = B * S
+    if not h.is_cuda or h.dtype not in (torch.bfloat16, torch.float16) or rows > DECODE_GEMV_ROWS:
+        return False
+    if getattr(model, "_duo_tp", False) or getattr(model, "_duo_seq", None) is not None:
+        return False
+    if hidden % 64 != 0 or rows * hidden > _C.GEMV_NORM_MAX_ELEMS:
+        return False
+    return all(_fusable(l) and l.mlp.down_proj.weight.shape[1] % 64 == 0 for l in model.model.layers)
+
+
+def _decode_gemv_forward(self, h, cos, sin, cache, rope_mode):
+    from .. import ops
+
+    base = self.model
+    layers = list(base.layers)
+    m = None
+    for idx, layer in enumerate(layers):
+        attn, mlp = layer.self_attn, layer.mlp
+        ln1, ln2 = layer.input_layernorm, layer.post_attention_layernorm
+        wqkv, bqkv = _qkv_weights(attn, h.device)
+        if m is None:
+            qkv, h = ops.gemv(h, wqkv, bqkv, norm_weight=ln1.weight, eps=ln1.variance_epsilon)
+        else:
+            qkv, h = ops.gemv(m, wqkv, bqkv, residual=h, norm_weight=ln1.weight, eps=ln1.variance_epsilon)
+        ctx = _attend(attn, qkv, cos, sin, cache, idx, rope_mode)
+        a = ops.gemv(ctx, attn.o_proj.weight, attn.o_proj.bias)
+        if getattr(mlp, "_duo_wgu", None) is None or mlp._duo_wgu.device != h.device:
+            _fuse_gate_up(mlp)
+        act, h = ops.gemv(a, mlp._duo_wgu, residual=h, norm_weight=ln2.weight, eps=ln2.variance_epsilon, silu=True)
+        m = ops.gemv(act, mlp.down_proj.weight, mlp.down_proj.bias)
+    if cache.dev_state is not None:
+        cache.advance_device(h.shape[1])
+    m_last, h_last = m[:, -1:, :].contiguous(), h[:, -1:, :].contiguous()
+    logits, _ = ops.gemv(m_last, self.lm_head.weight, self.lm_head.bias, residual=h_last, norm_weight=base.norm.weight,
+                         eps=base.norm.variance_epsilon, out_float=getattr(self, "_duo_logits_float", True))
+    return logits
 
 
 def _tp_layer_pipelined(layer, ctx, h, next_norm, group, n_blocks):
@@ -182,6 +235,9 @@
         cos, sin = base.rotary_emb(inputs_embeds, position_ids)
         cos, sin = cos[0].contiguous(), sin[0].contiguous()
     h = inputs_embeds.contiguous() if input_ids is not None else inputs_embeds.clone()
+    if decode_gemv_eligible(self, h):
+        logits = _decode_gemv_forward(self, h, cos, sin, cache, rope_mode)
+        return CausalLMOutputWithPast(logits=logits, past_key_values=cache if use_cache is not False else None)
     tp_on = getattr(self, "_duo_tp", False)
     seq_on = getattr(self, "_duo_seq", None) is not None
     if tp_on:
diff --git a/eval/efficiency/decode_breakdown.py b/eval/efficiency/decode_breakdown.py
--- /dev/null
+++ b/eval/efficiency/decode_breakdown.py
@@ -0,0 +1,183 @@
+from __future__ import annotations
+
+import argparse
+import json
+import os
+import subprocess
+import sys
+
+ROOT = os.path.dirname(os.path.dirname(os.path.dirname(os.path.abspath(__file__))))
+if ROOT not in sys.path:
+    sys.path.insert(0, ROOT)
+
+import torch
+
+import bench
+
+SITES = ("qkv", "o_proj", "gate_up", "down")
+
+
+def card():
+    try:
+        out = subprocess.run(["nvidia-smi", "--query-gpu=name,power.limit,clocks.max.sm", "--format=csv,noheader"],
+                             capture_output=True, text=True, timeout=30).stdout.strip().splitlines()[0]
+    except Exception as e:
+        out = f"nvidia-smi unavailable: {e!r}"
+    return out
+
+
+def read_ceiling(dev, gib=4, reps=10):
+    x = torch.ones(gib * (1 << 28), dtype=torch.float32, device=dev)
+    for _ in range(2):
+        x.sum()
+    e0, e1 = torch.cuda.Event(enable_timing=True), torch.cuda.Event(enable_timing=True)
+    e0.record()
+    for _ in range(reps):
+        x.sum()
+    e1.record()
+    torch.cuda.synchronize()
+    gbs = x.numel() * 4 * reps / (e0.elapsed_time(e1) / 1e3) / 1e9
+    del x
+    torch.cuda.empty_cache()
+    return gbs
+
+
+def site_bytes(model):
+    layers = model.model.layers
+    b = {s: 0 for s in SITES}
+    for l in layers:
+        a, m = l.self_attn, l.mlp
+        b["qkv"] += sum(p.weight.numel() for p in (a.q_proj, a.k_proj, a.v_proj)) * 2
+        b["o_proj"] += a.o_proj.weight.numel() * 2
+        b["gate_up"] += (m.gate_proj.weight.numel() + m.up_proj.weight.numel()) * 2
+        b["down"] += m.down_proj.weight.numel() * 2
+    b["lm_head"] = model.lm_head.weight.numel() * 2
+    return b
+
+
+def classify(events, n_layers, steps):
+    tot = {s: 0.0 for s in (*SITES, "lm_head", "attention", "glue")}
+    lin = []
+    for name, _, dur in events:
+        low = name.lower()
+        if "duo_attn" in low:
+            tot["attention"] += dur
+        elif "gemv" in low or "gemm" in low or "xmma" in low or "cutlass" in low or "cublas" in low:
+            lin.append(dur)
+        elif ("splitk" in low or "reduce_kernel" in low) and lin:
+            lin[-1] += dur
+        else:
+            tot["glue"] += dur
+    per_step = 4 * n_layers + 1
+    ok = len(lin) == per_step * steps
+    if ok:
+        for i, d in enumerate(lin):
+            j = i % per_step
+            tot["lm_head" if j == per_step - 1 else SITES[j % 4]] += d
+    else:
+        tot["glue"] += sum(lin)
+    return tot, ok, len(events)
+
+
+def profile(fn, steps):
+    from torch.profiler import ProfilerActivity, profile as tprof
+
+    fn()
+    torch.cuda.synchronize()
+    with tprof(activities=[ProfilerActivity.CUDA]) as prof:
+        for _ in range(steps):
+            fn()
+        torch.cuda.synchronize()
+    ev = [(e.name, e.time_range.start, e.time_range.end - e.time_range.start) for e in prof.events()
+          if e.device_type == torch.autograd.DeviceType.CUDA and "memcpy" not in e.name.lower()
+          and "memset" not in e.name.lower()]
+    ev.sort(key=lambda t: t[1])
+    return ev
+
+
+def main():
+    ap = argparse.ArgumentParser()
+    ap.add_argument("--ctx", type=int, default=524288)
+    ap.add_argument("--steps", type=int, default=20)
+    ap.add_argument("--prof-steps", type=int, default=3)
+    ap.add_argument("--out", default=None)
+    args = ap.parse_args()
+    dev = torch.device("cuda", 0)
+    torch.cuda.set_device(dev)
+    res = {"card": card(), "read_ceiling_gbs": read_ceiling(dev)}
+
+    from duo_attention_b200.graph import DuoDecodeGraph
+    from duo_attn.patch import DuoAttentionStaticKVCache
+
+    bargs = argparse.Namespace(arch="llama3-8b-1048k", layers=32, kv_format="bf16")
+    mask, _ = bench.head_pattern()
+    model, local_mask, _ = bench.build_model(bargs, mask, 0, 1, dev)
+    cache = DuoAttentionStaticKVCache(model, local_mask, 1, args.ctx + 8, bench.SINK, bench.RECENT,
+                                      prefilling_chunk_size=64)
+    bench.fill_cache_synthetic(cache, args.ctx)
+    tok = torch.zeros(1, 1, dtype=torch.long, device=dev)
+    L = len(model.model.layers)
+    wbytes = site_bytes(model)
+    wbytes["attention"] = bench.decode_bytes_per_token(local_mask, args.ctx)
+
+    def eager_step():
+        model(input_ids=tok, past_key_values=cache, use_cache=True)
+        cache.evict_last(1)
+
+    with torch.no_grad():
+        for _ in range(3):
+            eager_step()
+        ev_eager = profile(eager_step, args.prof_steps)
+        graph = DuoDecodeGraph(model, cache)
+
+        def graph_step():
+            graph.step(tok)
+            cache.evict_last(1)
+            graph.resync()
+
+        for _ in range(3):
+            graph_step()
+        torch.cuda.synchronize()
+        e0, e1 = torch.cuda.Event(enable_timing=True), torch.cuda.Event(enable_timing=True)
+        e0.record()
+        for _ in range(args.steps):
+            graph_step()
+        e1.record()
+        torch.cuda.synchronize()
+        step_ms = e0.elapsed_time(e1) / args.steps
+        ev_graph = profile(graph_step, args.prof_steps)
+
+    res["graph_step_ms"] = step_ms
+    res["weight_bytes_per_step"] = sum(v for k, v in wbytes.items() if k != "attention")
+    for tag, ev in (("graph", ev_graph), ("eager", ev_eager)):
+        tot, ok, n = classify(ev, L, args.prof_steps)
+        sites = {}
+        for s, us in tot.items():
+            ms = us / 1e3 / args.prof_steps
+            by = wbytes.get(s)
+            sites[s] = {"ms": ms, "bytes": by, "gbs": (by / (ms / 1e3) / 1e9) if by and ms else None}
+        kern_ms = sum(v["ms"] for v in sites.values())
+        span_ms = (ev[-1][1] + ev[-1][2] - ev[0][1]) / 1e3 / args.prof_steps if ev else 0.0
+        by_name = {}
+        for name, _, dur in ev:
+            c, t = by_name.get(name[:100], (0, 0.0))
+            by_name[name[:100]] = (c + 1, t + dur)
+        res[tag] = {"sites": sites, "kernel_ms_per_step": kern_ms, "kernels_per_step": n / args.prof_steps,
+                    "sites_classified": ok, "trace_span_ms_per_step": span_ms,
+                    "by_kernel": {k: {"per_step": c / args.prof_steps, "ms": t / 1e3 / args.prof_steps}
+                                  for k, (c, t) in sorted(by_name.items(), key=lambda kv: -kv[1][1])}}
+    g = res["graph"]
+    weights_ms = sum(g["sites"][s]["ms"] for s in (*SITES, "lm_head"))
+    res["graph"]["gap_ms_per_step"] = step_ms - g["kernel_ms_per_step"]
+    res["weights_plus_glue_plus_gaps_ms"] = step_ms - g["sites"]["attention"]["ms"]
+    res["weights_at_read_ceiling_ms"] = res["weight_bytes_per_step"] / (res["read_ceiling_gbs"] * 1e9) * 1e3
+    res["weights_kernel_ms"] = weights_ms
+    line = json.dumps(res, indent=1)
+    print(line)
+    if args.out:
+        with open(args.out, "w") as f:
+            f.write(line)
+
+
+if __name__ == "__main__":
+    main()
diff --git a/include/duo_b200.h b/include/duo_b200.h
--- a/include/duo_b200.h
+++ b/include/duo_b200.h
@@ -122,6 +122,15 @@
                             int64_t rows, int32_t hidden, float eps, int32_t dtype, void* stream);
 DUO_API int duo_silu_mul(const void* gate_up, void* out, int64_t rows, int32_t inter, int32_t dtype, void* stream);
 
+#define DUO_GEMV_NORM 2
+#define DUO_GEMV_SILU 1
+#define DUO_GEMV_F32_OUT 4
+#define DUO_GEMV_MAX_M 8
+DUO_API int duo_gemv(const void* x, const void* residual, const void* norm_weight, void* out_res, float eps,
+                     const void* w, const void* bias, void* y, int32_t m, int32_t n, int32_t k, int32_t flags,
+                     int32_t dtype, void* stream);
+DUO_API int duo_gemv_plan(int32_t m, int32_t n, int32_t k, int32_t flags, int32_t sm_count, int32_t* out);
+
 DUO_API int duo_attention_partial(const duo_layer* layer, int64_t n_keys, const void* q, int64_t q_row_stride,
                                   float* out_o, float* out_lse, int32_t q_len, float scale, void* workspace,
                                   size_t workspace_bytes, void* stream);
```

Result: slower. 43.92 (median of 6 runs) (-22.2%).
